# ariasanovsky/azdopt

Measured on AMD Instinct MI355X. Metric: node_expansions_per_s, higher is better.
Workload: dtype f32

## Files before the change

azdopt_amd/_lib.py:

```python
import ctypes as C
import os
import subprocess

_HERE = os.path.dirname(os.path.abspath(__file__))
LIB_PATH = os.environ.get("AZD_LIB", os.path.join(_HERE, "libazdopt_amd.so"))
_LIB = None

CTR = dict(EXPANSIONS=0, TERMINALS=1, TRANSPOSITIONS=2, VISITED_STEPS=3, SELECT_CALLS=4, SUM_DEG=5,
           SUM_ACTIONS=6, CASCADE_NODES=7, NEW_PREDS=8, ROOT_EXHAUSTED=9, MAX_FRONTIER=10, MAX_DEPTH=11,
           CURIOSITY_PAIRS=12, EVAL_LAYER_CLOCKS=13, TICKS_ADD_ACTIONS=14, FAILED=15, TICKS_TOTAL=16, TICKS_SELECT=17, TICKS_LOOKUP=18, TICKS_NEWNODE=19,
           TICKS_CASCADE=20, TICKS_MAX_CALL=21, TICKS_LAMBDA=22, TICKS_MATCHING=23, TICKS_WAIT=24, EVAL_BATCHES=25, EVAL_ROWS=26, EVAL_TILES=27, TICKS_TILES=28, TICKS_BATCH=29, TICKS_TILE_SETUP=30, TICKS_TILE_KLOOP=31)
CTR_COUNT = 32

ACT_NONE, ACT_RELU, ACT_SIGMOID = 0, 1, 2
ENGINE_NO_PERSISTENT_STEP = 1
ENGINE_ASYNC_STEP = 2
ENGINE_BARRIER_STEP = 4
ENGINE_POOL_STEP = 8
ENGINE_RAMSEY_U64 = 16
SPACE_C21 = 1
SPACE_RAMSEY = 2
SPACE_DENSE = 3
RAMSEY_MAX_N = 23
RAMSEY_WIDE_MAX_N = 32
# ... 57 lines not shown
    global _LIB
    if _LIB is not None:
        return _LIB
    if not os.path.exists(LIB_PATH):
        raise ImportError(f"{LIB_PATH} is missing: run __graft_entry__.build() (hipcc --offload-arch=gfx950); "
                          "azdopt_amd has no CPU fallback")
    L = C.CDLL(LIB_PATH)
    vp, i32p, u64p, f32p = C.c_void_p, C.POINTER(C.c_int32), C.POINTER(C.c_uint64), C.POINTER(C.c_float)

    def sig(name, res, *args):
        f = getattr(L, name, None)
        if f is None:
            if "AZD_LIB" in os.environ:
                return
            raise AttributeError("%s does not export %s" % (LIB_PATH, name))
        f.restype = res
        f.argtypes = list(args)

    sig("azd_status_string", C.c_char_p, C.c_int)
    sig("azd_last_error", C.c_char_p)
    sig("azd_version", C.c_int)
    sig("azd_device_count", C.c_int)
    sig("azd_c21_state_dim", C.c_int, C.c_int)
    sig("azd_c21_action_dim", C.c_int, C.c_int)
    sig("azd_c21_key_words", C.c_int, C.c_int)
    sig("azd_c21_generate_roots", C.c_int, C.c_uint64, C.c_uint64, C.c_uint64, C.c_int, C.c_int, C.c_int, C.c_int, vp, vp)
    sig("azd_evaluator_create_mlp", C.c_int, C.POINTER(vp), C.c_int, C.c_int, C.c_int, C.c_int, vp, C.c_int, C.c_int,
        C.POINTER(AdamConfig), C.c_uint64)
    sig("azd_evaluator_create_trivial", C.c_int, C.POINTER(vp), C.c_int, C.c_int, C.c_int)
    sig("azd_evaluator_create_hash_stream", C.c_int, C.POINTER(vp), C.c_int, C.c_int, C.c_int, C.c_uint64, C.c_uint64)
    sig("azd_evaluator_destroy", C.c_int, vp)
    sig("azd_evaluator_write_predictions", C.c_int, vp, C.c_int, vp, vp)
    sig("azd_evaluator_update_model", C.c_int, vp, C.c_int, vp, vp, vp, f32p)
    sig("azd_evaluator_write_predictions_dev", C.c_int, vp, C.c_int, vp, vp, vp)
    sig("azd_evaluator_update_model_dev", C.c_int, vp, C.c_int, vp, vp, vp, f32p, vp)
    sig("azd_evaluator_set_weight_storage", C.c_int, vp, C.c_int)
    sig("azd_evaluator_num_params", C.c_int64, vp)
    sig("azd_evaluator_get_params", C.c_int, vp, vp)
    sig("azd_evaluator_set_params", C.c_int, vp, vp)
    sig("azd_evaluator_calls", C.c_uint64, vp)
    sig("azd_engine_create", C.c_int, C.POINTER(vp), C.POINTER(EngineConfig), vp)
    sig("azd_engine_destroy", C.c_int, vp)
    sig("azd_engine_par_new", C.c_int, vp, vp, vp)
    sig("azd_engine_par_roll_out_episodes", C.c_int, vp, vp, C.c_int, C.c_uint32, C.c_int, i32p)
    sig("azd_engine_run_ahead", C.c_int, vp, vp, C.c_int, C.c_uint32, C.c_int, i32p)
    sig("azd_engine_par_update_model", C.c_int, vp, C.c_uint32, f32p)
    sig("azd_engine_par_update_model_sharded", C.c_int, vp, C.c_uint32, vp, f32p)
    sig("azd_engine_par_reset_trees", C.c_int, vp, vp, vp)
    sig("azd_engine_argmin_data", C.c_int, vp, C.POINTER(Argmin))
    sig("azd_engine_agent_counters", C.c_int, vp, vp)
    sig("azd_engine_agent_counters_per_agent", C.c_int, vp)
    sig("azd_engine_pool_agent_finish", C.c_int, vp, vp)
    sig("azd_engine_pool_groups", C.c_int, vp, vp, vp, vp)
    sig("azd_engine_ramsey_argmin_data", C.c_int, vp, C.POINTER(RamseyArgmin))
    sig("azd_engine_ramsey_wide_argmin_data", C.c_int, vp, C.POINTER(RamseyWideArgmin))
    sig("azd_engine_ramsey_argmin_any", C.c_int, vp, vp, C.c_int, vp, C.c_int, vp, f32p, i32p, C.POINTER(C.c_uint32))
    sig("azd_engine_ramsey_agent_counts", C.c_int, vp, C.c_int, vp, vp)
    sig("azd_ramsey_state_dim", C.c_int, C.c_int, C.c_int)
    sig("azd_ramsey_action_dim", C.c_int, C.c_int, C.c_int)
    sig("azd_ramsey_key_words", C.c_int, C.c_int, C.c_int)
    sig("azd_ramsey_generate_roots", C.c_int, C.c_uint64, C.c_uint64, C.c_uint64, C.c_int, C.c_int, C.c_int, C.c_int,
        C.c_int, vp, vp)
    sig("azd_dense_state_dim", C.c_int, C.c_int)
    sig("azd_dense_action_dim", C.c_int, C.c_int)
    sig("azd_dense_key_words", C.c_int, C.c_int)
    sig("azd_dense_generate_roots", C.c_int, C.c_uint64, C.c_uint64, C.c_uint64, C.c_int, C.c_int, C.c_int, C.c_int, C.c_double, vp, vp)
    sig("azd_engine_dense_argmin_data", C.c_int, vp, C.POINTER(DenseArgmin))
    sig("azd_c21_modify_roots", C.c_int, vp, C.c_uint64, C.c_uint64, C.c_int, C.c_int, vp, vp)
    sig("azd_c21_modify_roots_dev", C.c_int, vp, C.c_uint64, C.c_uint64, C.c_int, C.c_int, vp, vp)
    sig("azd_engine_par_reset_trees_c21", C.c_int, vp, C.c_uint64, C.c_uint64, C.c_int, C.c_int)
    sig("azd_engine_modify_roots_dev", C.c_int, vp, C.c_uint64, C.c_uint64, C.c_int, C.c_int, vp, vp)
    sig("azd_engine_par_reset_trees_policy", C.c_int, vp, C.c_uint64, C.c_uint64, C.c_int, C.c_int)
    sig("azd_engine_par_new_begin", C.c_int, vp, vp, vp)
    sig("azd_engine_par_new_end", C.c_int, vp, vp)
    sig("azd_engine_roll_out_begin", C.c_int, vp, vp, C.c_int, C.c_uint32)
    sig("azd_engine_roll_out_end", C.c_int, vp, vp, i32p)
    sig("azd_engine_reset_begin", C.c_int, vp, vp, vp)
    sig("azd_engine_reset_end", C.c_int, vp, vp)
    sig("azd_engine_observe", C.c_int, vp, C.c_uint32, vp, vp, vp)
    sig("azd_engine_observe_dev", C.c_int, vp, C.c_uint32, C.POINTER(vp), C.POINTER(vp), C.POINTER(vp))
    sig("azd_engine_read_state_vecs", C.c_int, vp, vp)
    sig("azd_engine_read_predictions", C.c_int, vp, vp)
    sig("azd_engine_debug_tile_forward", C.c_int, vp, vp, vp, C.c_int)
    sig("azd_engine_tree_sizes", C.c_int, vp, C.c_int, i32p, i32p, i32p)
    sig("azd_engine_export_tree", C.c_int, vp, C.c_int, *([vp] * 13))
    sig("azd_engine_agent_state", C.c_int, vp, C.c_int, vp, vp, vp, C.POINTER(C.c_uint32), C.POINTER(C.c_double), i32p)
    sig("azd_engine_counters", C.c_int, vp, vp)
    sig("azd_engine_set_timing", C.c_int, vp, C.c_int)
    sig("azd_engine_timing", C.c_int, vp, C.POINTER(C.c_double), C.POINTER(C.c_double), u64p)
    sig("azd_engine_stream", vp, vp)
    sig("azd_engine_step_form", C.c_int, vp, i32p, C.POINTER(C.c_char_p))
    sig("azd_engine_pool_split", C.c_int, vp, i32p, i32p)
    sig("azd_engine_pool_utilisation", C.c_int, vp, C.POINTER(C.c_double), C.POINTER(C.c_double))
    sig("azd_debug_probe_xcc", C.c_int, C.c_int, vp, C.c_int)
    sig("azd_debug_hash_stream_via_evaluators", C.c_int, vp, C.c_int)
    sig("azd_debug_mlp_gradients", C.c_int, vp, C.c_int, vp, vp, vp, vp, f32p)
    sig("azd_debug_probe_math", C.c_int, C.c_int, vp, vp, C.c_int)
    sig("azd_debug_gemm_bf16", C.c_int, C.c_int, C.c_int, C.c_int, C.c_int, vp, vp, vp, vp, C.c_int, C.c_int, C.c_int, C.c_int, f32p)
    sig("azd_debug_probe_cost", C.c_int, C.c_int, vp, C.c_int, C.c_int, C.c_int, C.c_int, vp, vp, f32p)
    _LIB = L
    return L


def check(status, where):
    if status != 0:
        raise AzdError(status, where)
# ... 5 lines not shown
```

azdopt_amd/csrc/engine.hip:

```cpp
#include <hip/hip_runtime.h>

#include <dlfcn.h>

#include <algorithm>
#include <cstdio>
#include <cstring>
#include <new>
#include <string>
#include <vector>

#include "../../include/azdopt_amd.h"
#include "c21_host.h"
#include "engine_types.h"
#include "evaluator.h"
#include "space_ops.h"

namespace azd {

thread_local std::string g_last_error;

int hip_fail(hipError_t e, const char *what) {
    g_last_error = std::string(what) + ": " + hipGetErrorString(e);
    if (e == hipErrorNoDevice || e == hipErrorInvalidDevice) return AZD_ERR_NO_DEVICE;
    if (e == hipErrorOutOfMemory) return AZD_ERR_OUT_OF_MEMORY;
// ... 112 lines not shown
    bool initialised = false;
    bool persist_enabled = true;
    bool barrier_step = false;
    azd::PersistArgs *d_pargs = nullptr;
    azd::PersistArgs *h_pargs = nullptr;
    azd::PersistArgs pargs_sent{};
    bool pargs_valid = false;
    bool log_clean = false;
    bool pool_clean = false;
    bool pool_failed = false;
    bool counters_by_wave = false;
    uint32_t *d_resume = nullptr;
    int16_t *d_grp_tile = nullptr;
    uint32_t *d_grp_lds = nullptr, *d_grp_desc = nullptr, *d_grp_cnt = nullptr, *d_grp_flag = nullptr;
    size_t grp_flag_words = 0;
    float *d_grp_x = nullptr;
    size_t grp_x_floats = 0, grp_slots_alloc = 0;
    std::vector<int16_t> grp_tile_host;
    std::vector<uint32_t> grp_lds_host;
    unsigned long long *d_log_key = nullptr;
    uint32_t *d_log_node = nullptr;
    int log_calls = 0;
    hipGraphExec_t call_graph = nullptr;
    azd::TolTable call_graph_tol{};
    uint64_t call_graph_layout = 0;
    bool graph_enabled = true;
    static constexpr int MAX_SUBS = 8;
    hipStream_t sub_stream[MAX_SUBS] = {};
    hipEvent_t sub_fork = nullptr, sub_join[MAX_SUBS] = {};
    hipGraphExec_t sub_graph[MAX_SUBS] = {};
    int sub_graph_n = 0;
    uint32_t *d_call_ctr = nullptr;
    static constexpr int EXT_STREAMS = 2;
    static constexpr int EXT_IN_FLIGHT = 4;
    hipStream_t ext_stream[EXT_STREAMS] = {};
    hipGraphExec_t ext_graph[EXT_STREAMS] = {};
    uint64_t ext_graph_layout = 0;
    int ext_graph_n = 0;
    bool ext_unsupported = false;
    uint32_t *d_ext_rows = nullptr, *d_ext_home = nullptr, *d_ext_n = nullptr;
    unsigned long long *d_ext_t0 = nullptr;
    int ext_depth = 2;
    hipEvent_t ext_done = nullptr, ext_fork = nullptr, ext_ring[EXT_STREAMS][EXT_IN_FLIGHT] = {};
    unsigned long long ext_iterations = 0;
    int kw_host = 0;
    int ramsey_slots = 0;
    int dense_slots = 0;
    uint64_t *d_stage_slots = nullptr;
    std::vector<uint64_t> dense_packed;
    std::vector<uint64_t> ramsey_perm_pad;
    bool pool_step = false;
    azd::PoolArgs pool{};
    size_t pool_slot_words = 0;
    int n_cus = 0;
    int pool_eval_wgs = 0, pool_search_wgs = 0;
    int pool_grp_g = 0, pool_grp_groups = 0, pool_grp_w = 0;
    int pool_search_waves = 0;
    double pool_util_eval = 0, pool_util_search = 0;
    struct {
        int n_eval = 0;
        int updates = 0;
    } pool_fb;
    struct Window {
        bool open = false;
        bool drained = false;
        bool lumped = false;
        int n = 0, consumed = 0;
        azd::TolTable tol{};
        uint32_t best_ord = 0;
        unsigned long long best_key = ~0ull;
        unsigned long long side_key = ~0ull;
        unsigned long long base_improved = 0;
        unsigned long long reported = 0;
        azd::FusedEval fe{};
        azd::PoolArgs pool{};
    } win;
    unsigned long long *h_win_log = nullptr;
    uint32_t *h_win_flag = nullptr;
    azd::ArgminRec *d_argmin_side = nullptr;
    azd::RamseyArgminRec *d_argmin_r_side = nullptr;
    bool ramsey_wide() const { return a.space == azd::SPACE_RAMSEY && a.KW > azd::MAX_KW; }
    bool ramsey_u64() const { return a.space == azd::SPACE_RAMSEY && a.KW == azd::RAMSEY_U64_KW; }
    size_t ramsey_nbr_words() const { return ramsey_u64() ? 512 : 128; }
    size_t argmin_r_bytes() const {
        return ramsey_u64() ? sizeof(azd::RamseyU64ArgminRec) : ramsey_wide() ? sizeof(azd::RamseyWideArgminRec) : sizeof(azd::RamseyArgminRec);
    }
    size_t argmin_r_recs() const { return (argmin_r_bytes() + sizeof(azd::RamseyArgminRec) - 1) / sizeof(azd::RamseyArgminRec); }
    float *d_pool = nullptr;
    size_t pool_rows = 0;
    int step_form = 0;
    std::string step_reason;

    template <typename T>
    int alloc(T **p, size_t count) {
        void *q = nullptr;
        hipError_t e = hipMalloc(&q, count * sizeof(T));
        if (e != hipSuccess) return azd::hip_fail(e, "hipMalloc");
        allocs.push_back(q);
        *p = (T *)q;
        return AZD_OK;
    }
    hipEvent_t get_event() {
        if (!ev_pool.empty()) {
            hipEvent_t e = ev_pool.back();
            ev_pool.pop_back();
            return e;
// ... 663 lines not shown
        TRY(e->alloc(&e->d_argmin_side, 1));
        if (ramsey) TRY(e->alloc(&e->d_argmin_r_side, e->argmin_r_recs()));
        hipError_t he3 = hipHostMalloc((void **)&e->h_win_log, (size_t)e->log_calls * sizeof(unsigned long long), hipHostMallocCoherent);
        if (he3 == hipSuccess) he3 = hipHostMalloc((void **)&e->h_win_flag, (size_t)e->log_calls * sizeof(uint32_t), hipHostMallocCoherent);
        if (he3 != hipSuccess) {
            st = azd::hip_fail(he3, "hipHostMalloc");
            azd_engine_destroy(e);
            return st;
        }
        e->pool.win_log = e->h_win_log;
        e->pool.win_flag = e->h_win_flag;
    }
    TRY(e->alloc(&e->d_stage_parents, B * (size_t)(dense ? 8 * a.n : ramsey ? a.E : a.n)));
    TRY(e->alloc(&e->d_stage_perm, B * (size_t)(dense ? 17 * a.KW : a.KW)));
    if (!dense) e->d_stage_slots = e->d_stage_perm;
    {
        hipError_t he = hipHostMalloc((void **)&e->h_status, sizeof(azd::StatusRec));
        if (he == hipSuccess) he = hipHostMalloc((void **)&e->h_argmin, sizeof(azd::ArgminRec));
        if (he != hipSuccess) {
            st = azd::hip_fail(he, "hipHostMalloc");
            azd_engine_destroy(e);
            return st;
        }
    }
    hipError_t he = hipMemsetAsync(a.counters, 0, B * azd::NUM_COUNTERS * 8, e->stream);
    if (he == hipSuccess) he = hipMemsetAsync(a.status, 0, sizeof(azd::StatusRec), e->stream);
    if (he == hipSuccess) he = hipMemsetAsync(a.argmin, 0, sizeof(azd::ArgminRec), e->stream);
    if (he == hipSuccess) he = hipMemsetAsync(a.flags, 0, B * 4, e->stream);
    if (he == hipSuccess) he = hipMemsetAsync(a.h_theta, 0, B * a.A * 4, e->stream);
    if (he == hipSuccess) he = hipMemsetAsync(a.state_vecs, 0, B * a.S * 4, e->stream);
    if (he == hipSuccess) he = hipMemsetAsync(a.weights, 0, B * a.A * 4, e->stream);
    if (he == hipSuccess) he = hipStreamSynchronize(e->stream);
    if (he != hipSuccess) {
        st = azd::hip_fail(he, "engine init memset");
        azd_engine_destroy(e);
        return st;
    }
#undef TRY
    *out = e;
    return AZD_OK;
}

int azd_engine_destroy(azd_engine *e) {
    if (!e) return AZD_OK;
    (void)hipSetDevice(e->cfg.device);
    if (e->stream) (void)hipStreamSynchronize(e->stream);
    for (void *p : e->allocs) (void)hipFree(p);
    if (e->h_status) (void)hipHostFree(e->h_status);
    if (e->h_argmin) (void)hipHostFree(e->h_argmin);
    if (e->h_pargs) (void)hipHostFree(e->h_pargs);
    if (e->h_win_log) (void)hipHostFree(e->h_win_log);
    if (e->h_win_flag) (void)hipHostFree(e->h_win_flag);
    if (e->d_pool) (void)hipFree(e->d_pool);
    for (void *p : {(void *)e->d_grp_tile, (void *)e->d_grp_lds, (void *)e->d_grp_desc, (void *)e->d_grp_cnt, (void *)e->d_grp_x, (void *)e->d_grp_flag})
        if (p) (void)hipFree(p);
    if (e->call_graph) (void)hipGraphExecDestroy(e->call_graph);
    for (int i = 0; i < azd_engine::MAX_SUBS; ++i) {
        if (e->sub_graph[i]) (void)hipGraphExecDestroy(e->sub_graph[i]);
        if (e->sub_join[i]) (void)hipEventDestroy(e->sub_join[i]);
        if (e->sub_stream[i]) (void)hipStreamDestroy(e->sub_stream[i]);
    }
    if (e->sub_fork) (void)hipEventDestroy(e->sub_fork);
    if (e->ext_done) (void)hipEventDestroy(e->ext_done);
    if (e->ext_fork) (void)hipEventDestroy(e->ext_fork);
    for (int x = 0; x < azd_engine::EXT_STREAMS; ++x) {
        if (e->ext_graph[x]) (void)hipGraphExecDestroy(e->ext_graph[x]);
        for (int i = 0; i < azd_engine::EXT_IN_FLIGHT; ++i)
            if (e->ext_ring[x][i]) (void)hipEventDestroy(e->ext_ring[x][i]);
        if (e->ext_stream[x]) (void)hipStreamDestroy(e->ext_stream[x]);
    }
    for (auto &it : e->ev_inflight) {
        (void)hipEventDestroy(it.second.first);
        (void)hipEventDestroy(it.second.second);
    }
    for (hipEvent_t ev : e->ev_pool) (void)hipEventDestroy(ev);
    if (e->stream) (void)hipStreamDestroy(e->stream);
    delete e;
    return AZD_OK;
}

int azd_engine_par_new_begin(azd_engine *e, const uint8_t *parents, const uint64_t *permitted) {
    if (!e || !parents || !permitted) return AZD_ERR_INVALID_ARGUMENT;
    AZD_ENTER(e);
    int st = upload_roots(e, parents, permitted);
    if (st) return st;
    const azd::Arenas &a = e->a;
    AZD_HIP(hipMemsetAsync(a.counters, 0, (size_t)a.B * azd::NUM_COUNTERS * 8, e->stream));
    e->counters_by_wave = false;
    AZD_HIP(hipMemsetAsync(a.status, 0, sizeof(azd::StatusRec), e->stream));
    e->seen_improved = 0;
    e->ops->init_roots(a, e->d_stage_parents, e->d_stage_perm, e->stream);
    AZD_HIP(hipMemsetAsync(a.h_theta, 0, (size_t)a.B * a.A * 4, e->stream));
    AZD_HIP(hipGetLastError());
    return AZD_OK;
}
static int new_finish(azd_engine *e) {
    e->ops->add_actions(e->a, 1, e->stream);
    e->ops->argmin(e->a, 1, e->stream);
    e->initialised = true;
    return sync_status(e);
}
int azd_engine_par_new_end(azd_engine *e, const float *h_theta) {
    if (!e || !h_theta) return AZD_ERR_INVALID_ARGUMENT;
    AZD_ENTER(e);
    AZD_HIP(hipMemcpyAsync(e->a.h_theta, h_theta, (size_t)e->a.B * e->a.A * 4, hipMemcpyHostToDevice, e->stream));
    return new_finish(e);
}
// ... 47 lines not shown
        tiles[l] = (fe.dims[l + 1] + 15) / 16;
        max_tiles = std::max(max_tiles, tiles[l]);
        if (l < L - 1) xs = std::max<uint32_t>(xs, (uint32_t)tiles[l] * 256u);
        if (l < L - 1 && fe.dims[l + 1] % 16 != 0) return false;
    }
    for (int W : {1, 2, 4})
    for (int g = force_g > 0 ? force_g : 8; g <= avail_wgs && g <= 128; g += 8) {
        {
            if (force_g <= 0 && W < 4 && 2 * g > avail_wgs) break;
            if ((max_tiles + g - 1) / g > W) {
                if (force_g > 0) break;
                continue;
            }
            struct Item { int l, t; size_t bytes; };
            std::vector<Item> items;
            for (int l = 0; l < L; ++l)
                for (int t = 0; t < tiles[l]; ++t) items.push_back({l, t, (size_t)steps[l] * 1024});
            std::stable_sort(items.begin(), items.end(), [](const Item &x, const Item &y) { return x.bytes > y.bytes; });
            std::vector<size_t> load((size_t)g, 0);
            std::vector<int> cnt((size_t)L * g, 0);
            std::vector<int16_t> tile((size_t)L * g * W, (int16_t)-1);
            std::vector<uint32_t> lds((size_t)L * g * W, 0u);
            bool ok = true;
            for (const Item &it : items) {
                int best = -1;
                for (int m = 0; m < g; ++m)
                    if (cnt[(size_t)it.l * g + m] < W && (best < 0 || load[(size_t)m] < load[(size_t)best])) best = m;
                if (best < 0 || load[(size_t)best] + it.bytes > lds_budget) {
                    ok = false;
                    break;
                }
                const int w = cnt[(size_t)it.l * g + best]++;
                tile[((size_t)it.l * g + best) * W + w] = (int16_t)it.t;
                lds[((size_t)it.l * g + best) * W + w] = (uint32_t)load[(size_t)best];
                load[(size_t)best] += it.bytes;
            }
            if (!ok) {
                if (force_g > 0) break;
                continue;
            }
            out->g = g;
            out->W = W;
            out->lds_bytes = *std::max_element(load.begin(), load.end());
            out->xstride = xs ? xs : 256u;
            out->tile = tile;
            out->lds = lds;
            return true;
        }
        if (force_g > 0) break;
    }
    return false;
}

static int pool_clear(azd_engine *e, const azd::PoolArgs &pool) {
    AZD_HIP(hipMemsetAsync(pool.ctl, 0, sizeof(azd::PoolCtl), e->stream));
    AZD_HIP(hipMemsetAsync(pool.ready_slots, 0, e->pool_slot_words * sizeof(uint32_t), e->stream));
    AZD_HIP(hipMemsetAsync(pool.join, 0, (size_t)e->a.B * sizeof(uint32_t), e->stream));
    e->pool_clean = true;
    return AZD_OK;
}

static int pool_finish_launch(azd_engine *e, const azd::FusedEval &fe, const azd::PoolArgs &pool, int k, bool *took_over,
                              uint32_t *as_out, size_t *ab_out) {
    *took_over = false;
    int st = fetch_status(e);
    if (st) return st;
    if (e->h_status->pool_ticks > 0 && !e->h_status->pool_abort) {
        const double T = (double)e->h_status->pool_ticks;
        e->pool_util_eval = e->pool_eval_wgs > 0 ? (double)e->h_status->pool_eval_busy / (T * e->pool_eval_wgs) : 0.0;
        e->pool_util_search = e->pool_search_waves > 0 ? (double)e->h_status->pool_search_busy / (T * e->pool_search_waves) : 0.0;
    }
    if (!e->h_status->pool_abort) return AZD_OK;
    e->pool_clean = false;
    e->log_clean = false;
    e->pool_failed = true;
    e->pool_step = false;
    uint32_t as = 0;
    size_t ab = 0;
    const char *why_t = "";
    if (!e->ops->async_plan(e->a, fe, &as, &ab, &why_t)) {
        e->time_collect();
        azd::g_last_error = std::string("pool step: a queue wait ran into its bound, and the asynchronous step cannot take over: ") + why_t;
        return AZD_ERR_UNREACHABLE;
    }
    azd::launch_pool_resume_scan(e->a, pool, k, e->d_resume, e->stream);
    st = pool_clear(e, pool);
    if (st) return st;
    azd::StepLaunch sl;
    sl.n_calls = k;
    sl.log_key = e->d_log_key;
    sl.resume = e->d_resume;
    sl.ctl = nullptr;
    sl.hashed = fe.kind == 4;
    sl.window = 0;
    e->time_begin(0);
    e->ops->launch_async(e->a, e->d_pargs, sl, fe.params, fe.wpk, as, ab, e->stream);
    e->time_end();
    e->log_clean = true;
    e->step_form = AZD_STEP_ASYNC;
    e->step_reason = "pool step aborted (a queue wait ran into its bound: no evaluator or searcher workgroup made progress); "
                     "the asynchronous step took the launch over and serves this engine from here on";
    *took_over = true;
    *as_out = as;
    *ab_out = ab;
    return AZD_OK;
}

static int dense_pool_run(azd_engine *e, const azd::TolTable &t, int n_calls, bool *ran, int *left_out) {
    *ran = false;
    *left_out = 0;
// ... 372 lines not shown
            if (const char *env = getenv("AZD_POOL_EVAL_GROUP")) {
                force_g = atoi(env);
                want = force_g > 0;
            }
            GroupPlan gpl;
            const int avail = capacity - n_search;
            if (want && plan_groups(fe, (size_t)160 * 1024 - 2048, avail, force_g, &gpl)) {
                const int n_groups = std::max(1, avail / gpl.g);
                const int NS = 16 / gpl.W;
                const size_t slots = (size_t)n_groups * NS;
                if (!e->d_grp_tile) {
                    AZD_HIP(hipMalloc(&e->d_grp_tile, (size_t)8 * 128 * 4 * sizeof(int16_t)));
                    AZD_HIP(hipMalloc(&e->d_grp_lds, (size_t)8 * 128 * 4 * sizeof(uint32_t)));
                }
                if (slots > e->grp_slots_alloc || slots * 2 * gpl.xstride > e->grp_x_floats || slots * gpl.g * 16 > e->grp_flag_words) {
                    AZD_HIP(hipStreamSynchronize(e->stream));
                    (void)hipFree(e->d_grp_desc);
                    (void)hipFree(e->d_grp_cnt);
                    (void)hipFree(e->d_grp_x);
                    (void)hipFree(e->d_grp_flag);
                    e->d_grp_flag = nullptr;
                    e->d_grp_desc = e->d_grp_cnt = nullptr;
                    e->d_grp_x = nullptr;
                    AZD_HIP(hipMalloc(&e->d_grp_desc, slots * 64 * 4));
                    AZD_HIP(hipMalloc(&e->d_grp_cnt, slots * 8 * 32 * 4));
                    AZD_HIP(hipMalloc(&e->d_grp_x, slots * 2 * gpl.xstride * 4));
                    AZD_HIP(hipMalloc(&e->d_grp_flag, slots * gpl.g * 16 * 4));
                    e->grp_flag_words = slots * gpl.g * 16;
                    e->grp_slots_alloc = slots;
                    e->grp_x_floats = slots * 2 * gpl.xstride;
                }
                if (gpl.tile != e->grp_tile_host || gpl.lds != e->grp_lds_host) {
                    AZD_HIP(hipStreamSynchronize(e->stream));
                    AZD_HIP(hipMemcpy(e->d_grp_tile, gpl.tile.data(), gpl.tile.size() * sizeof(int16_t), hipMemcpyHostToDevice));
                    AZD_HIP(hipMemcpy(e->d_grp_lds, gpl.lds.data(), gpl.lds.size() * sizeof(uint32_t), hipMemcpyHostToDevice));
                    e->grp_tile_host = gpl.tile;
                    e->grp_lds_host = gpl.lds;
                }
                pool.grp_g = gpl.g;
                pool.grp_w = gpl.W;
                pool.grp_groups = n_groups;
                pool.grp_tile = e->d_grp_tile;
                pool.grp_lds = e->d_grp_lds;
                pool.grp_desc = e->d_grp_desc;
                pool.grp_cnt = e->d_grp_cnt;
                pool.grp_x = e->d_grp_x;
                pool.grp_flag = e->d_grp_flag;
                pool.grp_xstride = gpl.xstride;
                n_eval = n_groups * gpl.g;
                pool.n_eval = n_eval;
                if (gpl.lds_bytes > dyn_bytes) dyn_bytes = gpl.lds_bytes;
            }
        }
        pool_blocks = n_eval + n_search;
        e->pool_grp_g = pool.grp_g;
        e->pool_grp_groups = pool.grp_groups;
        e->pool_grp_w = pool.grp_w;
        e->pool_eval_wgs = n_eval;
        e->pool_search_wgs = n_search;
        e->pool_search_waves = (n_search - pool.n_express) * 16 + pool.n_express * (int)pool.express_waves;
    }
    if (e->pool_step && fusable && !use_pool) {
        use_async = !e->barrier_step && e->ops->async_plan(e->a, fe, &dyn_stride, &dyn_bytes, &why_a);
        use_barrier = !use_async && e->ops->persist_plan(e->a, fe, &dyn_stride, &dyn_bytes, &why_b);
        if (!use_async) e->step_reason += why_a;
        if (!use_async && !use_barrier && *why_b) e->step_reason += std::string("; ") + why_b;
    }
    e->step_form = use_pool ? AZD_STEP_POOL : use_async ? AZD_STEP_ASYNC : use_barrier ? AZD_STEP_BARRIER : AZD_STEP_PER_CALL;
    if (e->a.space == azd::SPACE_DENSE)
        e->step_reason = dense_reason.empty() ? "AZD_DENSE_NO_POOL: the dense-graph space's pool step was switched off" : dense_reason;
    if (ahead) {
        const bool ok = use_pool && fe.kind >= 3 && n_calls >= 1 && n_calls <= e->log_calls && !e->timing;
        if (!ok) return AZD_OK;
        *accepted = 1;
    }
    if (use_pool || use_async || use_barrier) {
        auto send_args = [&](const azd::PoolArgs &pl) -> int {
            azd::PersistArgs &pa = e->pargs_sent;
            azd::PersistArgs now;
            memset(&now, 0, sizeof(now));
            now.a = e->a;
            now.tol = t;
            now.ev = fe;
            now.ev.call_base = (fe.kind == 2 || fe.kind == 4) ? e->ev->calls : 0;
            now.pool = pl;
            if (e->pargs_valid && memcmp(&pa, &now, sizeof(now)) == 0) return AZD_OK;
            AZD_HIP(hipStreamSynchronize(e->stream));
            memcpy(e->h_pargs, &now, sizeof(now));
            AZD_HIP(hipMemcpyAsync(e->d_pargs, e->h_pargs, sizeof(azd::PersistArgs), hipMemcpyHostToDevice, e->stream));
            memcpy(&pa, &now, sizeof(now));
            e->pargs_valid = true;
            return AZD_OK;
        };
        const bool fb_on = use_pool && fe.kind == 3 && pool_feedback_on() && n_calls >= 100 && !getenv("AZD_POOL_EVAL_WGS");
        int left = n_calls;
        while (left > 0) {
            const int k = left < e->log_calls ? left : e->log_calls;
            status_fresh = false;
            st = send_args(pool);
            if (st) return st;
            if (use_pool && !e->pool_clean) {
                st = pool_clear(e, pool);
                if (st) return st;
            }
            if (use_pool && pool.grp_g > 0) {
                const size_t slots = (size_t)pool.grp_groups * (16 / pool.grp_w);
// ... 658 lines not shown
    return AZD_OK;
}
int azd_engine_ramsey_agent_counts(azd_engine *e, int agent, int32_t *counts, int32_t *totals) {
    if (!e || agent < 0 || agent >= e->a.B) return AZD_ERR_INVALID_ARGUMENT;
    if (e->a.space != azd::SPACE_RAMSEY) return AZD_ERR_UNSUPPORTED;
    AZD_ENTER(e);
    AZD_HIP(hipStreamSynchronize(e->stream));
    const azd::Arenas &a = e->a;
    if (counts) AZD_HIP(hipMemcpy(counts, a.cur_counts + (size_t)agent * a.C * a.E, (size_t)a.C * a.E * 4, hipMemcpyDeviceToHost));
    if (totals) AZD_HIP(hipMemcpy(totals, a.cur_tot + (size_t)agent * 4, 16, hipMemcpyDeviceToHost));
    return AZD_OK;
}

int azd_engine_argmin_data(azd_engine *e, azd_argmin *out) {
    if (!e || !out || !e->initialised) return AZD_ERR_INVALID_ARGUMENT;
    if (e->a.space != azd::SPACE_C21) return AZD_ERR_UNSUPPORTED;
    AZD_HIP(hipSetDevice(e->cfg.device));
    bool side = false;
    {
        const int st_w = window_argmin_side(e, &side);
        if (st_w) return st_w;
    }
    static_assert(sizeof(azd_argmin) == sizeof(azd::ArgminRec), "ABI struct mismatch");
    AZD_HIP(hipMemcpyAsync(e->h_argmin, side ? e->d_argmin_side : e->a.argmin, sizeof(azd::ArgminRec), hipMemcpyDeviceToHost, e->stream));
    AZD_HIP(hipStreamSynchronize(e->stream));
    memcpy(out, e->h_argmin, sizeof(azd_argmin));
    return AZD_OK;
}

int azd_engine_read_state_vecs(azd_engine *e, float *out) {
    if (!e || !out) return AZD_ERR_INVALID_ARGUMENT;
    AZD_ENTER(e);
    AZD_HIP(hipStreamSynchronize(e->stream));
    AZD_HIP(hipMemcpy(out, e->a.state_vecs, (size_t)e->a.B * e->a.S * 4, hipMemcpyDeviceToHost));
    return AZD_OK;
}
int azd_engine_debug_tile_forward(azd_engine *e, const float *states, float *predictions, int rows) {
    if (!e || !states || !predictions || rows < 1) return AZD_ERR_INVALID_ARGUMENT;
    AZD_ENTER(e);
    azd::FusedEval fe;
    azd::PoolArgs pool = e->pool;
    uint32_t dyn_stride = 0;
    size_t dyn_bytes = 0;
    const char *why = "";
    if (e->a.space == azd::SPACE_DENSE || !e->ev->fused_desc(&fe) || fe.kind != 3 || !e->ops->pool_plan(e->a, fe, &pool, &dyn_stride, &dyn_bytes, &why)) {
        azd::g_last_error = "debug_tile_forward: needs the c21 or the Ramsey space with an MLP evaluator the pool step can serve";
        return AZD_ERR_INVALID_ARGUMENT;
    }
    float *d_in = nullptr, *d_out = nullptr;
    hipError_t he = hipMalloc(&d_in, (size_t)rows * e->a.S * 4);
    const char *what = "hipMalloc";
    if (he == hipSuccess) he = hipMalloc(&d_out, (size_t)rows * e->a.A * 4);
    if (he == hipSuccess) what = "hipMemcpyAsync", he = hipMemcpyAsync(d_in, states, (size_t)rows * e->a.S * 4, hipMemcpyHostToDevice, e->stream);
    if (he == hipSuccess) what = "k_tile_forward", he = azd::launch_tile_forward(fe, pool, rows, d_in, d_out, e->stream);
    if (he == hipSuccess) what = "hipMemcpyAsync", he = hipMemcpyAsync(predictions, d_out, (size_t)rows * e->a.A * 4, hipMemcpyDeviceToHost, e->stream);
    if (he == hipSuccess) what = "hipStreamSynchronize", he = hipStreamSynchronize(e->stream);
    else (void)hipStreamSynchronize(e->stream);
    (void)hipFree(d_in);
    (void)hipFree(d_out);
    return he == hipSuccess ? AZD_OK : azd::hip_fail(he, what);
}
int azd_engine_read_predictions(azd_engine *e, float *out) {
    if (!e || !out) return AZD_ERR_INVALID_ARGUMENT;
    AZD_ENTER(e);
    AZD_HIP(hipStreamSynchronize(e->stream));
    AZD_HIP(hipMemcpy(out, e->a.h_theta, (size_t)e->a.B * e->a.A * 4, hipMemcpyDeviceToHost));
    return AZD_OK;
}

int azd_engine_tree_sizes(azd_engine *e, int agent, int *n_nodes, int *n_arcs, int *n_preds) {
    if (!e || agent < 0 || agent >= e->a.B) return AZD_ERR_INVALID_ARGUMENT;
    AZD_ENTER(e);
    AZD_HIP(hipStreamSynchronize(e->stream));
    uint32_t v[3];
    AZD_HIP(hipMemcpy(&v[0], e->a.n_nodes + agent, 4, hipMemcpyDeviceToHost));
    AZD_HIP(hipMemcpy(&v[1], e->a.n_arcs + agent, 4, hipMemcpyDeviceToHost));
    AZD_HIP(hipMemcpy(&v[2], e->a.n_preds + agent, 4, hipMemcpyDeviceToHost));
    if (n_nodes) *n_nodes = (int)v[0];
    if (n_arcs) *n_arcs = (int)v[1];
    if (n_preds) *n_preds = (int)v[2];
    return AZD_OK;
}

int azd_engine_export_tree(azd_engine *e, int agent, float *c, float *c_star, uint32_t *n_t, uint32_t *exhausted,
                           uint32_t *act_begin, uint32_t *act_end, uint64_t *keys, uint32_t *arc_src,
                           uint32_t *arc_dst, uint32_t *arc_pp, uint32_t *pred_a_id, float *pred_g,
                           int32_t *pred_arc) {
    int nn, na, np;
    int st = azd_engine_tree_sizes(e, agent, &nn, &na, &np);
    if (st) return st;
    const azd::Arenas &a = e->a;
    std::vector<azd::NodeRec> nodes((size_t)nn);
    std::vector<azd::ArcRec> arcs((size_t)na);
    std::vector<azd::PredRec> preds((size_t)np);
    AZD_HIP(hipMemcpy(nodes.data(), a.nodes + (size_t)agent * a.node_cap, nodes.size() * sizeof(azd::NodeRec), hipMemcpyDeviceToHost));
    if (na) AZD_HIP(hipMemcpy(arcs.data(), a.arcs + (size_t)agent * a.arc_cap, arcs.size() * sizeof(azd::ArcRec), hipMemcpyDeviceToHost));
    if (np) AZD_HIP(hipMemcpy(preds.data(), a.preds + (size_t)agent * a.pred_cap, preds.size() * sizeof(azd::PredRec), hipMemcpyDeviceToHost));
    std::vector<float> g_exp((size_t)np);
    if (np) AZD_HIP(hipMemcpy(g_exp.data(), a.pred_g + (size_t)agent * a.pred_cap, g_exp.size() * 4, hipMemcpyDeviceToHost));
    if (keys && a.space == azd::SPACE_DENSE) {
        const int KW = a.KW, MAXS = e->dense_slots;
        std::vector<uint64_t> rk((size_t)nn * KW);
        std::vector<uint16_t> tab((size_t)MAXS);
        AZD_HIP(hipMemcpy(rk.data(), a.keys + (size_t)agent * a.node_cap * KW, rk.size() * 8, hipMemcpyDeviceToHost));
        AZD_HIP(hipMemcpy(tab.data(), a.root_aid + (size_t)agent * MAXS, tab.size() * 2, hipMemcpyDeviceToHost));
        memset(keys, 0, (size_t)nn * e->kw_host * 8);
        for (int i = 0; i < nn; ++i)
// ... 95 lines not shown
    if (!e || !out) return AZD_ERR_INVALID_ARGUMENT;
    AZD_ENTER(e);
    AZD_HIP(hipStreamSynchronize(e->stream));
    const azd::Arenas &a = e->a;
    std::vector<unsigned long long> h((size_t)a.B * azd::NUM_COUNTERS);
    std::vector<uint32_t> fl((size_t)a.B);
    AZD_HIP(hipMemcpy(h.data(), a.counters, h.size() * 8, hipMemcpyDeviceToHost));
    AZD_HIP(hipMemcpy(fl.data(), a.flags, fl.size() * 4, hipMemcpyDeviceToHost));
    for (int k = 0; k < AZD_CTR_COUNT; ++k) out[k] = 0;
    for (int i = 0; i < a.B; ++i) {
        for (int k = 0; k < azd::NUM_COUNTERS; ++k) {
            unsigned long long v = h[(size_t)i * azd::NUM_COUNTERS + k];
            if (k >= AZD_CTR_COUNT) continue;
            if (k == AZD_CTR_MAX_FRONTIER || k == AZD_CTR_MAX_DEPTH || k == AZD_CTR_TICKS_MAX_CALL) out[k] = std::max<uint64_t>(out[k], v);
            else out[k] += v;
        }
    }
    uint64_t failed = 0;
    for (uint32_t f : fl) failed += f != 0;
    out[AZD_CTR_FAILED_AGENTS] = failed;
    return AZD_OK;
}

int azd_engine_agent_counters(azd_engine *e, uint64_t *out) {
    if (!e || !out) return AZD_ERR_INVALID_ARGUMENT;
    AZD_ENTER(e);
    AZD_HIP(hipStreamSynchronize(e->stream));
    AZD_HIP(hipMemcpy(out, e->a.counters, (size_t)e->a.B * azd::NUM_COUNTERS * 8, hipMemcpyDeviceToHost));
    return AZD_OK;
}
int azd_engine_agent_counters_per_agent(azd_engine *e) { return e ? (e->counters_by_wave ? 0 : 1) : AZD_ERR_INVALID_ARGUMENT; }

int azd_engine_set_timing(azd_engine *e, int enabled) {
    if (!e) return AZD_ERR_INVALID_ARGUMENT;
    e->timing = enabled != 0;
    e->rollout_ms = e->evaluator_ms = 0;
    e->rollout_launches = 0;
    return AZD_OK;
}
int azd_engine_timing(azd_engine *e, double *tree_ms, double *evaluator_ms, uint64_t *tree_launches) {
    if (!e) return AZD_ERR_INVALID_ARGUMENT;
    if (tree_ms) *tree_ms = e->rollout_ms;
    if (evaluator_ms) *evaluator_ms = e->evaluator_ms;
    if (tree_launches) *tree_launches = e->rollout_launches;
    return AZD_OK;
}
void *azd_engine_stream(azd_engine *e) { return e ? (void *)e->stream : nullptr; }
int azd_engine_pool_utilisation(azd_engine *e, double *eval_busy, double *search_busy) {
    if (!e) return AZD_ERR_INVALID_ARGUMENT;
    if (eval_busy) *eval_busy = e->pool_util_eval;
    if (search_busy) *search_busy = e->pool_util_search;
    return AZD_OK;
}
int azd_engine_pool_groups(azd_engine *e, int *members, int *groups, int *waves_per_slot) {
    if (!e) return AZD_ERR_INVALID_ARGUMENT;
    if (members) *members = e->pool_grp_g;
    if (groups) *groups = e->pool_grp_groups;
    if (waves_per_slot) *waves_per_slot = e->pool_grp_w;
    return AZD_OK;
}
int azd_engine_pool_agent_finish(azd_engine *e, uint64_t *ticks_out) {
    if (!e || !ticks_out) return AZD_ERR_INVALID_ARGUMENT;
    AZD_ENTER(e);
    if (!e->pool.stamp) {
        azd::g_last_error = "pool_agent_finish: this engine has run no pool step";
        return AZD_ERR_INVALID_ARGUMENT;
    }
    AZD_HIP(hipStreamSynchronize(e->stream));
    AZD_HIP(hipMemcpy(ticks_out, e->pool.stamp, (size_t)e->a.B * 8, hipMemcpyDeviceToHost));
    return AZD_OK;
}
int azd_engine_pool_split(azd_engine *e, int *eval_wgs, int *search_wgs) {
    if (!e) return AZD_ERR_INVALID_ARGUMENT;
    if (eval_wgs) *eval_wgs = e->pool_eval_wgs;
    if (search_wgs) *search_wgs = e->pool_search_wgs;
    return AZD_OK;
}
int azd_debug_probe_xcc(int device, uint32_t *out, int n_blocks) {
    if (!out || n_blocks <= 0) return AZD_ERR_INVALID_ARGUMENT;
    int st = azd::device_ok(device);
    if (st) return st;
    AZD_HIP(hipSetDevice(device));
    uint32_t *d = nullptr;
    AZD_HIP(hipMalloc(&d, (size_t)n_blocks * 4));
    azd::launch_probe_xcc(d, n_blocks, nullptr);
    hipError_t he = hipDeviceSynchronize();
    if (he == hipSuccess) he = hipMemcpy(out, d, (size_t)n_blocks * 4, hipMemcpyDeviceToHost);
    (void)hipFree(d);
    if (he != hipSuccess) return azd::hip_fail(he, "probe_xcc");
    return AZD_OK;
}
int azd_engine_step_form(azd_engine *e, int *form, const char **reason) {
    if (!e) return AZD_ERR_INVALID_ARGUMENT;
    if (form) *form = e->step_form;
    if (reason) *reason = e->step_reason.c_str();
    return AZD_OK;
}

int azd_debug_probe_math(int device, const float *in, float *out, int n) {
    if (!in || !out || n <= 0) return AZD_ERR_INVALID_ARGUMENT;
    int st = azd::device_ok(device);
    if (st) return st;
    AZD_HIP(hipSetDevice(device));
    float *d_in = nullptr, *d_out = nullptr;
    AZD_HIP(hipMalloc(&d_in, (size_t)n * 8));
    AZD_HIP(hipMalloc(&d_out, (size_t)n * 16));
// ... 149 lines not shown
```

azdopt_amd/csrc/engine_types.h:

```cpp
#pragma once
#include <stddef.h>
#include <stdint.h>

namespace azd {

constexpr uint32_t NONE = 0xFFFFFFFFu;
constexpr int PARENTS_STRIDE = 32;
constexpr int MAX_N = 24;
constexpr int MAX_KW = 6;
constexpr int PATH_SET = 0, PATH_SEQUENCE = 1;
constexpr int SPACE_C21 = 1, SPACE_RAMSEY = 2, SPACE_DENSE = 3;
constexpr int PRED_CHUNKS = 2;
constexpr int MAX_NODE_ACTIONS = 64 * PRED_CHUNKS;
constexpr int RAMSEY_U64_KW = 36;
constexpr int RAMSEY_U64_CH = 8;
constexpr int FRONTIER_CAP = 256;
constexpr int PATH_STACK = 32;
constexpr int MAX_TOL = 32;
constexpr int NUM_COUNTERS = 32;

struct __attribute__((aligned(16))) NodeRec {
    float c_star;
    uint32_t nt_ex;
    float c;
// ... 162 lines not shown
struct FusedEval {
    int kind;
    uint64_t seed, first_agent, call_base;
    const float *params;
    int n_layers;
    int dims[8];
    int final_act;
    int max_hidden;
    int hid[2];
    long long w_off[7], b_off[7];
    int bf16;
    const uint16_t *w16;
    const void *wpk;
    long long p_off[7];
};

struct TolTable {
    uint32_t tol[MAX_TOL];
    int n_tol;
    uint32_t tol_default;
};

constexpr int POOL_XCDS = 8;
struct PoolQ {
    uint32_t head, pad0[31];
    uint32_t tail, pad1[31];
};
struct PoolCtl {
    uint32_t claim_next, pad0[31];
    uint32_t done_agents, pad1[31];
    uint32_t abort, pad2[31];
    PoolQ ready[2][POOL_XCDS];
    PoolQ evalq[2][POOL_XCDS];
    struct {
        uint32_t v, pad[31];
    } sum_calls[POOL_XCDS], claimed[POOL_XCDS],
      done_x[POOL_XCDS],
      max_lag[POOL_XCDS];
    unsigned long long eval_busy;
    unsigned long long search_busy;
    unsigned long long t_first;
    unsigned long long t_last;
};
struct PendRec {
    uint32_t pos;
    float c;
    uint32_t n_preds;
    uint32_t call;
};
struct PoolArgs {
    PoolCtl *ctl;
    uint32_t *ready_slots;
    uint32_t *eval_slots;
    int ready_lanes;
    int n_express;
    uint32_t express_waves;
    uint32_t express_shift;
    int early_post;
    uint32_t qcap;
    uint32_t *join;
    PendRec *pend;
    unsigned long long *stamp;
    int n_eval;
    uint32_t eval_stride;
    uint32_t eval_out_off;
    uint32_t eval_rows;
    uint32_t *post_call;
    int grp_g, grp_w, grp_groups;
    const int16_t *grp_tile;
    const uint32_t *grp_lds;
    uint32_t *grp_desc;
    uint32_t *grp_cnt;
    uint32_t *grp_flag;
    float *grp_x;
    uint32_t grp_xstride;
    uint32_t debug_abort_call;
    uint32_t *win_count;
    unsigned long long *win_log;
    uint32_t *win_flag;
};

struct StepLaunch {
    int n_calls;
    unsigned long long *log_key;
    const uint32_t *resume;
    PoolCtl *ctl;
    int hashed;
    int groups = 0;
    int window;
};

struct PersistArgs {
    Arenas a;
    TolTable tol;
    FusedEval ev;
    PoolArgs pool;
};

}
```

azdopt_amd/csrc/pool_kernels.hip:

```cpp
#define AZD_TU_ASYNC 1
#define AZD_TU_POOL 1
#include <hip/hip_runtime.h>

#include "bf16.h"
#include "c21_host.h"
#include "space_ops.h"

namespace azd {

#include "tree_core.inc"
#include "space_c21.inc"
#include "persistent_step.inc"
#include "async_step.inc"
#include "pool_step.inc"
#include "launchers.inc"

static bool e_pool_plan(const Arenas &a, const FusedEval &ev, PoolArgs *pool, uint32_t *dyn_stride, size_t *dyn_bytes, const char **why) {
    return pool_plan_common(a, ev, pool, dyn_stride, dyn_bytes, why, C21Space<1>::pool_dyn_bytes(a), sizeof(WaveLds));
}
static void e_launch_pool(const Arenas &a, const PersistArgs *d_args, const StepLaunch &sl, const float *params,
                          const void *wpk, int n_blocks, uint32_t dyn_stride, size_t dyn_bytes, void *stream) {
    DISPATCH_KW(a, l_pool, a, d_args, sl, params, wpk, n_blocks, dyn_stride, dyn_bytes, (hipStream_t)stream);
}
static int e_pool_max_resident(const Arenas &a, size_t dyn_bytes, int n_cus) {
    int nb = 0;
    DISPATCH_KW(a, q_pool_resident, &nb, dyn_bytes);
    return nb * n_cus;
}
const PoolOps &c21_pool_ops() {
    static const PoolOps ops = {e_pool_plan, e_launch_pool, e_pool_max_resident};
    return ops;
}

__global__ __launch_bounds__(PERSIST_WAVES * 64) void k_tile_forward(const FusedEval ev, const float *__restrict__ params, const void *__restrict__ wpk,
                                                                     const uint32_t stride, const uint32_t out_off, const int n_rows,
                                                                     const float *__restrict__ states, float *__restrict__ out) {
    __shared__ uint32_t agents[PERSIST_WAVES];
    const int tid = threadIdx.x, wave = tid >> 6, first = blockIdx.x * PERSIST_WAVES;
    const int n = n_rows - first < PERSIST_WAVES ? n_rows - first : PERSIST_WAVES;
    const int S = ev.dims[0], S16 = (S + 15) & ~15, L = ev.n_layers, A = ev.dims[L];
    if (tid < PERSIST_WAVES) agents[tid] = (uint32_t)(first + tid);
    PoolRows rows;
    rows.stride = stride;
    rows.out_off = out_off;
    rows.agents = agents;
    rows.n = n;
    EvalPtrs gp;
    gp.params = params;
    gp.wpk = wpk;
    gp.state_vecs = states;
    gp.h_theta = out;
    for (int idx = tid; idx < n * S16; idx += PERSIST_WAVES * 64) {
        const int r = idx / S16, c = idx - r * S16;
        const float v = c < S ? states[(size_t)(first + r) * S + c] : 0.f;
        if (ev.bf16) reinterpret_cast<uint16_t *>(rows.row(r))[c] = (uint16_t)bf16_bits(v);
        else rows.row(r)[c] = v;
    }
    __syncthreads();
    for (int l = 0; l < L; ++l) {
        const int nt = (ev.dims[l + 1] + 15) >> 4;
        for (int tile = wave; tile < nt; tile += PERSIST_WAVES) {
            unsigned long long ph[3];
            mlp_tile_task<PoolRows, true>(ev, rows, gp, l, tile, ph);
        }
        __syncthreads();
    }
    for (int idx = tid; idx < n * A; idx += PERSIST_WAVES * 64) {
        const int r = idx / A, c = idx - r * A;
        out[(size_t)(first + r) * A + c] = rows.out(r)[c];
    }
}
hipError_t launch_tile_forward(const FusedEval &ev, const PoolArgs &pool, int n_rows, const float *states, float *out, void *stream) {
    const size_t dyn_bytes = (size_t)pool.eval_stride * sizeof(float) * PERSIST_WAVES;
    hipError_t he = hipFuncSetAttribute((const void *)k_tile_forward, hipFuncAttributeMaxDynamicSharedMemorySize, (int)dyn_bytes);
    if (he != hipSuccess) return he;
    k_tile_forward<<<dim3((n_rows + PERSIST_WAVES - 1) / PERSIST_WAVES), dim3(PERSIST_WAVES * 64), dyn_bytes, (hipStream_t)stream>>>(
        ev, ev.params, ev.wpk, pool.eval_stride, pool.eval_out_off, n_rows, states, out);
    return hipGetLastError();
}
__global__ void k_pool_resume_scan(Arenas a, const PendRec *__restrict__ pend, const uint32_t *__restrict__ claim_next, const int n_calls,
                                   uint32_t *__restrict__ resume) {
    const int t = blockIdx.x * blockDim.x + threadIdx.x;
    if (t >= a.B) return;
    const uint32_t claimed = *claim_next;
    uint32_t r = 0u;
    if ((uint32_t)t < claimed) {
        const NodeRec nd = a.nodes[(size_t)t * a.node_cap + a.state_pos[t]];
        const bool pending = a.flags[t] == 0u && nd.act_end == 0u;
        r = pending ? (pend[t].call | 0x80000000u) : (uint32_t)n_calls;
    }
    resume[t] = r;
}
void launch_pool_resume_scan(const Arenas &a, const PoolArgs &pool, int n_calls, uint32_t *resume, void *stream) {
    k_pool_resume_scan<<<dim3((a.B + 255) / 256), dim3(256), 0, (hipStream_t)stream>>>(a, pool.pend, &pool.ctl->claim_next, n_calls, resume);
}
__global__ void k_probe_xcc(uint32_t *out) {
    if (threadIdx.x == 0) out[blockIdx.x] = pool_xcc_id();
}
void launch_probe_xcc(uint32_t *d_out, int n_blocks, void *stream) {
    k_probe_xcc<<<dim3(n_blocks), dim3(64), 0, (hipStream_t)stream>>>(d_out);
}

}
```

azdopt_amd/csrc/pool_step.inc:

```

constexpr unsigned long long POOL_WAIT_TICKS = 400000000ull;
struct PoolWait {
    unsigned long long t0;
    uint32_t polls;
    __device__ __forceinline__ PoolWait() : t0(0), polls(0) {}
    __device__ __forceinline__ bool expired() {
        if ((++polls & 255u) != 0u) return false;
        const unsigned long long now = (unsigned long long)wall_clock64();
        if (t0 == 0) t0 = now;
        return now - t0 > POOL_WAIT_TICKS;
    }
};

__device__ __forceinline__ uint32_t pool_xcc_id() {
    uint32_t v;
    asm volatile("s_getreg_b32 %0, hwreg(HW_REG_XCC_ID)" : "=s"(v));
    return v & 7u;
}

#ifndef AZD_POOL_FILL_WAIT
#define AZD_POOL_FILL_WAIT 2
#endif
#ifndef AZD_POOL_FILL_SLEEP
#define AZD_POOL_FILL_SLEEP 32
// ... 135 lines not shown
__device__ __forceinline__ int opaque_lane() {
    int v;
    asm volatile("v_mbcnt_lo_u32_b32 %0, -1, 0\n\tv_mbcnt_hi_u32_b32 %0, -1, %0" : "=v"(v));
    return v;
}
__device__ __forceinline__ void pool_tile1(const FusedEval &ev, const PoolRows &rows, const EvalPtrs &gp, const int l, const int tile) {
    const int L = ev.n_layers;
    const int K = ev.dims[l], N = ev.dims[l + 1];
    const int S4 = (ev.dims[0] + 15) & ~15, H = ev.hid[0];
    const int nrows = rows.count();
    const int n0 = tile * 16;
    const int steps = (K + 15) >> 4;
    const size_t tile0 = (size_t)ev.p_off[l] + (size_t)tile * steps * 256;
    azd_tile_acc acc = {0.f, 0.f, 0.f, 0.f};
    {
        const int lane = opaque_lane();
        const int r = lane & 15;
        float *const rbase = rows.row(r < nrows ? r : 0);
        const int in_off = (l == 0 ? 0 : S4 + ((l - 1) & 1) * H) + 4 * (lane >> 4);
        if (ev.bf16)
            tile_k_loop_bf16(acc, reinterpret_cast<const uint16_t *>(gp.wpk) + tile0, (uint32_t)lane * 8u,
                             (uint32_t)(uintptr_t)(reinterpret_cast<const uint16_t *>(rbase) + in_off), steps);
        else
            tile_k_loop_f32(acc, reinterpret_cast<const float *>(gp.wpk) + tile0, (uint32_t)lane * 16u, (uint32_t)(uintptr_t)(rbase + in_off), steps);
    }
    const int lane = opaque_lane();
    const int col = n0 + (lane & 15);
    if (col < N) {
        const float bj = gp.params[ev.b_off[l] + col];
        const int act = (l == L - 1) ? ev.final_act : 1;
#pragma unroll
        for (int i = 0; i < 4; ++i) {
            const int row = 4 * (lane >> 4) + i;
            if (row < nrows) {
                const float v = act_apply(acc[i] + bj, act);
                if (l == L - 1) rows.out(row)[col] = v;
                else if (ev.bf16) reinterpret_cast<uint16_t *>(rows.row(row))[S4 + (l & 1) * H + col] = (uint16_t)bf16_bits(v);
                else rows.row(row)[S4 + (l & 1) * H + col] = v;
            }
        }
    }
}

__device__ __forceinline__ void pool_hash_rows(const FusedEval &ev, const PoolArgs &pl, const PoolBatch &bt, const PoolRows &rows, const int n,
                                            const int A) {
    for (int idx = threadIdx.x; idx < n * A; idx += PERSIST_WAVES * 64) {
        const int r = idx / A, i = idx - r * A;
        const uint64_t agent = ev.first_agent + (uint64_t)bt.agent[r], cidx = ev.call_base + (uint64_t)ld_sc1(pl.post_call + bt.agent[r]);
        const uint64_t h = splitmix(splitmix(splitmix(splitmix(ev.seed ^ 0x70726564ull) ^ agent) ^ cidx) ^ (uint64_t)i);
        rows.out(r)[i] = (float)(h >> 40) * (1.0f / 16777216.0f);
    }
}

template <bool HASHED>
__device__ __forceinline__ void pool_eval(const PersistArgs *pa, const EvalPtrs &gp, PoolBatch &bt, const uint32_t xcc) {
    const Arenas &a = pa->a;
    const FusedEval &ev = pa->ev;
    const PoolArgs &pl = pa->pool;
    PoolCtl *ctl = pl.ctl;
    const int tid = threadIdx.x, wave = tid >> 6;
    const uint32_t B = (uint32_t)a.B, qmask = pl.qcap - 1u;
    constexpr bool hashed = HASHED;
    const int S = ev.dims[0], S16 = (S + 15) & ~15, L = hashed ? 0 : ev.n_layers, A = hashed ? a.A : ev.dims[L];
    PoolRows rows;
    rows.stride = pl.eval_stride;
    rows.out_off = pl.eval_out_off;
    rows.agents = bt.agent;
    unsigned long long n_batches = 0, n_rows = 0, n_tiles = 0, busy = 0, t_stage = 0, t_layers = 0, c_layers = 0;
    for (;;) {
        if (tid == 0) {
            uint32_t n = 0, first0 = 0, first1 = 0, cnt0 = 0, cnt1 = 0, q = 0, leave = 0;
            PoolWait wt;
            int fill_waits = AZD_POOL_FILL_WAIT;
            for (;;) {
                for (uint32_t k = 0; k < (uint32_t)POOL_XCDS && n == 0u; ++k) {
                    const uint32_t x = (xcc + k) & (uint32_t)(POOL_XCDS - 1);
                    const uint32_t h0 = AZD_POOL_PRIORITY ? ld_sc1(&ctl->evalq[0][x].head) : 0u, t0 = AZD_POOL_PRIORITY ? ld_sc1(&ctl->evalq[0][x].tail) : 0u;
                    const uint32_t h1 = ld_sc1(&ctl->evalq[1][x].head), t1 = ld_sc1(&ctl->evalq[1][x].tail);
                    const int a0 = (int)(t0 - h0) > 0 ? (int)(t0 - h0) : 0, a1 = (int)(t1 - h1) > 0 ? (int)(t1 - h1) : 0;
                    if (a0 + a1 == 0) continue;
                    const int cap = ((int)pl.eval_rows > PERSIST_WAVES && a0 + a1 >= (int)pl.eval_rows) ? (int)pl.eval_rows : PERSIST_WAVES;
                    if (a0 == 0 && a1 < PERSIST_WAVES && fill_waits > 0) {
                        --fill_waits;
                        __builtin_amdgcn_s_sleep(AZD_POOL_FILL_SLEEP);
                        k = (uint32_t)POOL_XCDS;
                        continue;
                    }
                    uint32_t c0 = 0, c1 = 0;
                    if (a0 > 0) {
                        const uint32_t take = a0 < cap ? (uint32_t)a0 : (uint32_t)cap;
                        if (atomicCAS(&ctl->evalq[0][x].head, h0, h0 + take) == h0) c0 = take;
                    }
                    if (a1 > 0 && c0 < (uint32_t)cap) {
                        const uint32_t room = (uint32_t)cap - c0;
                        const uint32_t take = (uint32_t)a1 < room ? (uint32_t)a1 : room;
                        if (atomicCAS(&ctl->evalq[1][x].head, h1, h1 + take) == h1) c1 = take;
                    }
                    if (c0 + c1) {
                        n = c0 + c1;
                        first0 = h0;
                        first1 = h1;
                        cnt0 = c0;
                        cnt1 = c1;
                        q = x;
                    } else k = (uint32_t)POOL_XCDS;
                }
                if (n) break;
                if (ld_sc1(&ctl->done_agents) >= B || ld_sc1(&ctl->abort) != 0u) {
                    leave = 1;
                    break;
                }
                __builtin_amdgcn_s_sleep(AZD_POOL_EVAL_IDLE_SLEEP);
                if (wt.expired()) {
                    atomicExch(&ctl->abort, 1u);
                    leave = 1;
                    break;
                }
            }
            bt.n = n;
            bt.first[0] = first0;
            bt.first[1] = first1;
            bt.cnt[0] = cnt0;
            bt.cnt[1] = cnt1;
            bt.q = q;
            bt.leave = leave;
        }
        __syncthreads();
        if (bt.leave) break;
        const int n = (int)bt.n;
        const unsigned long long tb0 = (unsigned long long)wall_clock64();
        if (tid < n) {
            const uint32_t lane_q = (uint32_t)tid < bt.cnt[0] ? 0u : 1u;
            const uint32_t ticket = lane_q == 0u ? bt.first[0] + (uint32_t)tid : bt.first[1] + (uint32_t)tid - bt.cnt[0];
            uint32_t *slot = pl.eval_slots + ((size_t)lane_q * POOL_XCDS + bt.q) * pl.qcap + (ticket & qmask);
            uint32_t v = 0;
            PoolWait wt;
            while ((v = ld_sc1(slot)) == 0u) {
                __builtin_amdgcn_s_sleep(1);
                if (wt.expired() || ld_sc1(&ctl->abort) != 0u) {
                    atomicExch(&ctl->abort, 1u);
                    bt.leave = 1u;
                    break;
                }
            }
            st_sc1(slot, 0u);
            bt.agent[tid] = v ? (v & 0xFFFFFFu) - 1u : 0u;
            bt.home[tid] = v >> 24;
#ifdef AZD_PHASE_PROFILE
            if (v) {
                unsigned long long *st = pl.stamp + bt.agent[tid];
                atomicAdd(&a.counters[(size_t)bt.agent[tid] * NUM_COUNTERS + 24], (unsigned long long)wall_clock64() - __hip_atomic_load(st, __ATOMIC_RELAXED, __HIP_MEMORY_SCOPE_AGENT));
            }
#endif
        }
        __syncthreads();
        if (bt.leave) break;
        rows.n = n;
        if (hashed) pool_hash_rows(ev, pl, bt, rows, n, A);
        else {
            const int q4 = S16 >> 2;
            for (int idx = tid; idx < n * q4; idx += PERSIST_WAVES * 64) {
                const int r = idx / q4, c4 = idx - r * q4;
                azd_f32x4 v = {0.f, 0.f, 0.f, 0.f};
                if (4 * c4 < S) v = ld_sc1_x4(gp.state_vecs + (size_t)bt.agent[r] * S + 4 * c4);
                if (ev.bf16) {
                    uint16_t *d = reinterpret_cast<uint16_t *>(rows.row(r)) + 4 * c4;
                    d[0] = (uint16_t)bf16_bits(v[0]);
                    d[1] = (uint16_t)bf16_bits(v[1]);
                    d[2] = (uint16_t)bf16_bits(v[2]);
                    d[3] = (uint16_t)bf16_bits(v[3]);
                } else *reinterpret_cast<azd_f32x4 *>(rows.row(r) + 4 * c4) = v;
            }
        }
        __syncthreads();
        const unsigned long long tb1 = (unsigned long long)wall_clock64();
        const unsigned long long cb1 = (unsigned long long)__builtin_amdgcn_s_memtime();
        for (int l = 0; l < L; ++l) {
            const int nt = (ev.dims[l + 1] + 15) >> 4;
            for (int tile = wave; tile < nt; tile += PERSIST_WAVES) {
                if (n > PERSIST_WAVES) {
                    if (ev.bf16) pool_tile2<true>(ev, rows, gp, l, tile);
                    else pool_tile2<false>(ev, rows, gp, l, tile);
                } else {
#if AZD_POOL_ASM_TILE
                    pool_tile1(ev, rows, gp, l, tile);
#else
                    unsigned long long ph[3];
                    mlp_tile_task<PoolRows, true>(ev, rows, gp, l, tile, ph);
#endif
                }
            }
            __syncthreads();
        }
        for (int l = 0; l < L; ++l) n_tiles += (unsigned long long)((ev.dims[l + 1] + 15) >> 4);
        const unsigned long long tb2 = (unsigned long long)wall_clock64();
        t_stage += tb1 - tb0;
        t_layers += tb2 - tb1;
        c_layers += (unsigned long long)__builtin_amdgcn_s_memtime() - cb1;
        {
            const int a4 = A >> 2;
            for (int idx = tid; idx < n * a4; idx += PERSIST_WAVES * 64) {
                const int r = idx / a4, c4 = idx - r * a4;
                st_sc1_x4(gp.h_theta + (size_t)bt.agent[r] * A + 4 * c4, *reinterpret_cast<const azd_f32x4 *>(rows.out(r) + 4 * c4));
            }
        }
        VM_DRAIN();
        __syncthreads();
        if (tid < n && ((bt.home[tid] & 0x40u) == 0u || (atomicAdd(&pl.join[bt.agent[tid]], 1u) & 1u))) {
#ifdef AZD_PHASE_PROFILE
            __hip_atomic_store(pl.stamp + bt.agent[tid], (unsigned long long)wall_clock64(), __ATOMIC_RELAXED, __HIP_MEMORY_SCOPE_AGENT);
#endif
            const uint32_t x = bt.home[tid] & (uint32_t)(POOL_XCDS - 1);
            const uint32_t rl = (pl.ready_lanes && (bt.home[tid] & 0x80u)) ? 0u : 1u;
            const uint32_t i = atomicAdd(&ctl->ready[rl][x].tail, 1u);
            st_sc1(pl.ready_slots + ((size_t)rl * POOL_XCDS + x) * pl.qcap + (i & qmask), bt.agent[tid] + 1u);
        }
        n_batches += 1;
        n_rows += (unsigned long long)n;
        if (tid == 0 && blockIdx.x == 0 && pl.debug_abort_call != 0u && n_batches == (unsigned long long)pl.debug_abort_call) atomicExch(&ctl->abort, 1u);
        busy += (unsigned long long)wall_clock64() - tb0;
    }
    if (tid == 0) {
        atomicAdd(&ctl->eval_busy, busy);
        atomicMax(&ctl->t_last, (unsigned long long)wall_clock64());
        unsigned long long *ctr = a.counters + (size_t)(blockIdx.x % (uint32_t)a.B) * NUM_COUNTERS;
        atomicAdd(&ctr[25], n_batches);
        atomicAdd(&ctr[26], n_rows);
// ... 250 lines not shown
                if (v >= gen && v != 0xFFFFFFFFu) break;
                __builtin_amdgcn_s_sleep(2);
                if (wt.expired() || ((wt.polls & 63u) == 0u && ld_sc1(&ctl->abort) != 0u)) {
                    atomicExch(&ctl->abort, 1u);
                    leave = true;
                    break;
                }
            }
            if (leave) {
                tell_all(7, 0xFFFFFFFFu);
                break;
            }
            n_batches += 1;
            n_rows += (unsigned long long)n;
            for (int l = 0; l < L; ++l) n_tiles += (unsigned long long)((ev.dims[l + 1] + 15) >> 4);
            busy += (unsigned long long)wall_clock64() - tb0;
            if (lane == 0 && si == 0 && pl.debug_abort_call != 0u && n_batches == (unsigned long long)pl.debug_abort_call) atomicExch(&ctl->abort, 1u);
        }
    }
    if (leader && lane == 0) {
        atomicAdd(&ctl->eval_busy, busy);
        atomicMax(&ctl->t_last, (unsigned long long)wall_clock64());
        unsigned long long *ctr = a.counters + (size_t)((blockIdx.x * PERSIST_WAVES + (uint32_t)wave) % (uint32_t)a.B) * NUM_COUNTERS;
        atomicAdd(&ctr[25], n_batches);
        atomicAdd(&ctr[26], n_rows);
        atomicAdd(&ctr[27], n_tiles);
        atomicAdd(&ctr[29], busy);
    }
}

struct PoolIdle {
    uint32_t leave;
    uint32_t claims_done;
    uint32_t mean_calls;
};

__device__ __forceinline__ void pool_window_count(const PoolArgs &pl, const unsigned long long *log_key, const uint32_t call, const uint32_t B) {
    if (atomicAdd(pl.win_count + call, 1u) + 1u != B) return;
    const unsigned long long key = __hip_atomic_load(log_key + call, __ATOMIC_RELAXED, __HIP_MEMORY_SCOPE_AGENT);
    __hip_atomic_store(pl.win_log + call, key, __ATOMIC_RELAXED, __HIP_MEMORY_SCOPE_SYSTEM);
    __hip_atomic_store(pl.win_flag + call, 1u, __ATOMIC_RELEASE, __HIP_MEMORY_SCOPE_SYSTEM);
}

template <class SP, int MODE>
__device__ __forceinline__ void pool_search(const PersistArgs *pa, const int n_calls, unsigned long long *__restrict__ log_key, typename SP::Lds &s,
                            const uint32_t dyn, const uint32_t xcc, PoolIdle &idle, const bool express) {
    const Arenas &a = pa->a;
    const TolTable &tol = pa->tol;
    const FusedEval &ev = pa->ev;
    const PoolArgs &pl = pa->pool;
    PoolCtl *ctl = pl.ctl;
    constexpr bool HASHED = (MODE & 1) != 0, WINDOW = (MODE & 2) != 0;
    const uint32_t B = (uint32_t)a.B, qmask = pl.qcap - 1u;
    uint32_t *rslots[2] = {pl.ready_slots + (size_t)xcc * pl.qcap, pl.ready_slots + ((size_t)POOL_XCDS + xcc) * pl.qcap};
    uint32_t *eslots[2] = {pl.eval_slots + (size_t)xcc * pl.qcap, pl.eval_slots + ((size_t)POOL_XCDS + xcc) * pl.qcap};
    for (;;) {
#ifdef AZD_WAVE_PHASES
        const unsigned long long wp_take0 = PH_NOW();
#endif
        uint32_t t = NONE, pending = 0, waited = 0;
        if (LANE == 0) {
            if (!express && LDS_LOAD(&idle.claims_done) == 0u) {
                const uint32_t c = atomicAdd(&ctl->claim_next, 1u);
                if (c < B) {
                    t = c;
                    atomicAdd(&ctl->claimed[xcc].v, 1u);
#ifdef AZD_PHASE_PROFILE
                    a.counters[(size_t)c * NUM_COUNTERS + 31] = (unsigned long long)wall_clock64();
#endif
                } else LDS_STORE(&idle.claims_done, 1u);
            }
            if (t == NONE && LDS_LOAD(&idle.leave) == 0u) {
                uint32_t rl = 1u;
                if (pl.ready_lanes == 1 && (int)(ld_sc1(&ctl->ready[0][xcc].head) - ld_sc1(&ctl->ready[0][xcc].tail)) < AZD_POOL_STANDBY) rl = 0u;
                if (express) rl = 0u;
                else if (pl.ready_lanes == 2 && (int)(ld_sc1(&ctl->ready[0][xcc].tail) - ld_sc1(&ctl->ready[0][xcc].head)) > 0) rl = 0u;
                const uint32_t h = atomicAdd(&ctl->ready[rl][xcc].head, 1u);
                uint32_t *slot = rslots[rl] + (h & qmask);
                PoolWait wt;
                uint32_t v = 0, polls = 0, seen_progress = 0xFFFFFFFFu;
                while ((v = ld_sc1(slot)) == 0u) {
                    if ((++polls & 15u) == 0u) {
                        if (LDS_LOAD(&idle.leave) != 0u) break;
                        if (ld_sc1(&ctl->done_agents) >= B || ld_sc1(&ctl->abort) != 0u) {
                            LDS_STORE(&idle.leave, 1u);
                            break;
                        }
                    }
                    __builtin_amdgcn_s_sleep(AZD_POOL_POLL_SLEEP);
#ifdef AZD_POOL_POLL_SLEEP2
                    __builtin_amdgcn_s_sleep(AZD_POOL_POLL_SLEEP2);
#endif
                    if (wt.expired()) {
                        uint32_t progress = 0u;
                        for (int x = 0; x < POOL_XCDS; ++x) progress += ld_sc1(&ctl->sum_calls[x].v);
                        if (progress != seen_progress) {
                            seen_progress = progress;
                            wt = PoolWait();
                        } else {
                            atomicExch(&ctl->abort, 1u);
                            LDS_STORE(&idle.leave, 1u);
                            break;
                        }
                    }
                }
                if (v) {
                    st_sc1(slot, 0u);
                    if ((h & 7u) == 0u || express) {
// ... 10 lines not shown
            }
        }
        t = uni(t);
        pending = uni(pending);
        waited = uni(waited);
        if (t == NONE) break;
        __builtin_amdgcn_fence(__ATOMIC_ACQUIRE, "agent");
#ifdef AZD_PHASE_PROFILE
        if (LANE < 24) s.ctr[LANE] = 0;
#endif
        if (LANE == 0) s.ctr[31] = (unsigned long long)wall_clock64();
#ifdef AZD_WAVE_PHASES
        CTR_ADD(24, PH_NOW() - wp_take0);
        const unsigned long long wp_add0 = PH_NOW();
#endif
        WAVE_SYNC();
        uint32_t call = 0u;
        RolloutOut first;
        first.first_nact = 0u;
        if (pending) {
#ifdef AZD_PHASE_PROFILE
            CTR_ADD(28, (unsigned long long)wall_clock64() - __hip_atomic_load(pl.stamp + t, __ATOMIC_RELAXED, __HIP_MEMORY_SCOPE_AGENT));
#endif
            const PendRec pr = pl.pend[t];
            RolloutOut ro;
            ro.flags = 0;
            ro.cand_c = 0.f;
            ro.cand_node = NONE;
            ro.pos = pr.pos;
            ro.c = pr.c;
            ro.n_preds = pr.n_preds;
            call = pr.call;
            add_actions_agent<SP, true>(a, s, (int)t, 0, &ro, &first);
#ifdef AZD_WAVE_PHASES
            CTR_ADD(14, PH_NOW() - wp_add0);
#endif
        }
        bool posted = false;
        for (;; ++call) {
            if (call >= (uint32_t)n_calls) {
                if (LANE == 0) {
                    atomicAdd(&ctl->done_agents, 1u);
                    if (pl.ready_lanes == 2) atomicAdd(&ctl->done_x[xcc].v, 1u);
#ifdef AZD_PHASE_PROFILE
                    a.counters[(size_t)t * NUM_COUNTERS + 30] = (unsigned long long)wall_clock64();
#else
                    pl.stamp[t] = (unsigned long long)wall_clock64() - __hip_atomic_load(&ctl->t_first, __ATOMIC_RELAXED, __HIP_MEMORY_SCOPE_AGENT);
#endif
                }
                break;
            }
            RolloutOut ro;
            ro.post_tail = nullptr;
            ro.posted = 0u;
            ro.known_live = first.first_nact != 0u ? 1u : 0u;
            ro.first_nact = first.first_nact;
            ro.first_pp = first.first_pp;
            ro.first_aid = first.first_aid;
            ro.first_g = first.first_g;
            first.first_nact = 0u;
            uint32_t behind = 0u, lane_q = 1u;
            if (HASHED || ev.kind == 3) {
#if AZD_POOL_PRIORITY
                {
                    const uint32_t cl = ld_sc1(&ctl->claimed[xcc].v);
                    const uint32_t mean = ld_sc1(&ctl->sum_calls[xcc].v) / (cl ? cl : 1u);
                    const uint32_t slack = (mean >> 5) > 2u ? (mean >> 5) : 2u;
                    if (call + 1u + slack < mean) lane_q = 0u;
                }
#endif
                if (pl.ready_lanes == 2) {
                    const uint32_t ref = LDS_LOAD(&idle.mean_calls);
                    if (call + (uint32_t)AZD_POOL_EXPRESS_SLACK + (ref >> pl.express_shift) < ref) behind = 0x80u;
                } else if (pl.ready_lanes) {
                    const uint32_t cl = ld_sc1(&ctl->claimed[xcc].v);
                    const uint32_t mean = ld_sc1(&ctl->sum_calls[xcc].v) / (cl ? cl : 1u);
                    behind = call + 1u + (uint32_t)AZD_POOL_READY_SLACK < mean ? 0x80u : 0u;
                }
                bool early = pl.early_post == 1;
                if (pl.early_post == 2) {
                    const uint32_t mean = LDS_LOAD(&idle.mean_calls);
                    early = waited || behind != 0u || call + (uint32_t)AZD_POOL_BEHIND_SLACK + (mean >> AZD_POOL_BEHIND_SHIFT) < mean;
                }
                ro.post_tail = early ? &ctl->evalq[lane_q][xcc].tail : nullptr;
                ro.post_slots = eslots[lane_q];
                ro.post_mask = qmask;
                ro.post_word = (t + 1u) | ((xcc | behind | 0x40u) << 24);
                ro.post_stamp = pl.stamp + t;
                if (HASHED && LANE == 0) st_sc1(pl.post_call + t, call);
            }
#ifdef AZD_WAVE_PHASES
            const unsigned long long wp_roll0 = PH_NOW();
#endif
            const bool expanded = rollout_agent<SP, true, true>(a, tol, s, dyn, (int)t, &ro);
#ifdef AZD_WAVE_PHASES
            CTR_ADD(28, PH_NOW() - wp_roll0);
#endif
            if (LANE == 0 && ro.flags == 0) {
                const uint32_t node = ro.cand_node;
                if (node != NONE) {
                    const unsigned long long key = ((unsigned long long)ordf(ro.cand_c) << 32) |
                                                   ((unsigned long long)(t & 0xFFFFu) << 16) | (unsigned long long)(node & 0xFFFFu);
                    atomicMin(&log_key[call], key);
                    a.cand_node[t] = NONE;
                }
            }
            if (LANE == 0) atomicAdd(&ctl->sum_calls[xcc].v, 1u);
            if (!expanded) {
                if (WINDOW) {
                    VM_DRAIN();
                    if (LANE == 0) pool_window_count(pl, log_key, call, B);
                }
                continue;
            }
            if (HASHED || ev.kind == 3) {
                if (LANE == 0) {
                    PendRec pr;
                    pr.pos = ro.pos;
                    pr.c = ro.c;
                    pr.n_preds = ro.n_preds;
                    pr.call = call + 1u;
                    pl.pend[t] = pr;
                }
                WAVE_SYNC();
                POOL_FLUSH_PER_AGENT(a, s, (int)t);
                VM_DRAIN();
                if (LANE == 0) {
                    if (!ro.posted) {
#ifdef AZD_PHASE_PROFILE
                        __hip_atomic_store(pl.stamp + t, (unsigned long long)wall_clock64(), __ATOMIC_RELAXED, __HIP_MEMORY_SCOPE_AGENT);
#endif
                        const uint32_t i = atomicAdd(&ctl->evalq[lane_q][xcc].tail, 1u);
                        st_sc1(eslots[lane_q] + (i & qmask), (t + 1u) | ((xcc | behind) << 24));
                    }
                    else if (atomicAdd(&pl.join[t], 1u) & 1u) {
#ifdef AZD_PHASE_PROFILE
                        __hip_atomic_store(pl.stamp + t, (unsigned long long)wall_clock64(), __ATOMIC_RELAXED, __HIP_MEMORY_SCOPE_AGENT);
#endif
                        const uint32_t rl = (pl.ready_lanes && behind) ? 0u : 1u;
                        const uint32_t i = atomicAdd(&ctl->ready[rl][xcc].tail, 1u);
                        st_sc1(rslots[rl] + (i & qmask), t + 1u);
                    }
                    if (WINDOW) pool_window_count(pl, log_key, call, B);
                }
                posted = true;
                break;
            }
            if (ev.kind == 2) {
                float *h = a.h_theta + (size_t)t * a.A;
                const uint64_t agent = ev.first_agent + (uint64_t)t, cidx = ev.call_base + (uint64_t)call;
                for (int i = LANE; i < a.A; i += 64) {
                    uint64_t r = splitmix(splitmix(splitmix(splitmix(ev.seed ^ 0x70726564ull) ^ agent) ^ cidx) ^ (uint64_t)i);
                    h[i] = (float)(r >> 40) * (1.0f / 16777216.0f);
                }
                WAVE_SYNC();
            }
            add_actions_agent<SP, false>(a, s, (int)t, 0, &ro, &first);
        }
        if (!posted) {
            WAVE_SYNC();
            POOL_FLUSH_PER_AGENT(a, s, (int)t);
        }
        if (LANE == 0) s.ctr[30] += (unsigned long long)wall_clock64() - s.ctr[31];
    }
    if (LANE == 0) {
        atomicAdd(&ctl->search_busy, s.ctr[30]);
        atomicMax(&ctl->t_last, (unsigned long long)wall_clock64());
    }
#ifndef AZD_PHASE_PROFILE
    WAVE_SYNC();
#ifdef AZD_WAVE_PHASES
    if ((LANE == 24 || LANE == 28) && s.ctr[LANE]) atomicAdd(&a.counters[(size_t)((blockIdx.x * PERSIST_WAVES + (threadIdx.x >> 6)) % B) * NUM_COUNTERS + LANE], s.ctr[LANE]);
#endif
    if (LANE < 24) {
        const unsigned long long v = s.ctr[LANE];
        unsigned long long *ctr = a.counters + (size_t)((blockIdx.x * PERSIST_WAVES + (threadIdx.x >> 6)) % B) * NUM_COUNTERS;
        if (LANE == 10 || LANE == 11 || LANE == 21) atomicMax(&ctr[LANE], v);
        else if (v) atomicAdd(&ctr[LANE], v);
    }
#endif
#ifdef AZD_PHASE_PROFILE
    if (LANE == 0 && s.ctr[28]) atomicAdd(&a.counters[(size_t)((blockIdx.x * PERSIST_WAVES + (threadIdx.x >> 6)) % B) * NUM_COUNTERS + 28], s.ctr[28]);
#endif
}

template <class SP, int MODE>
__global__ __launch_bounds__(PERSIST_WAVES * 64) void k_pool(const PersistArgs *__restrict__ pa, int n_calls,
                                                             unsigned long long *__restrict__ log_key, uint32_t dyn_stride,
                                                             const float *__restrict__ params, const float *state_vecs,
                                                             float *h_theta, const void *__restrict__ wpk) {
    constexpr uint32_t SW_BYTES = (uint32_t)((PERSIST_WAVES * sizeof(typename SP::Lds) + 15) & ~(size_t)15);
    typename SP::Lds *const sw = reinterpret_cast<typename SP::Lds *>(lds_base(0u));
    __shared__ PoolBatch bt;
    __shared__ PoolIdle idle;
    const uint32_t xcc = pool_xcc_id();
    if (threadIdx.x == 0) atomicCAS(&pa->pool.ctl->t_first, 0ull, (unsigned long long)wall_clock64());
    if ((int)blockIdx.x < pa->pool.n_eval) {
        EvalPtrs gp;
        gp.params = params;
        gp.wpk = wpk;
        gp.state_vecs = state_vecs;
        gp.h_theta = h_theta;
        if constexpr ((MODE & 4) != 0) {
            if (pa->pool.grp_g > 0 && (int)blockIdx.x < pa->pool.grp_groups * pa->pool.grp_g) {
                pool_eval_group(pa, gp, xcc);
                return;
            }
        }
        pool_eval<(MODE & 1) != 0>(pa, gp, bt, xcc);
        return;
    }
    const int wave = threadIdx.x >> 6;
    typename SP::Lds &s = sw[wave];
    if (threadIdx.x == 0) {
        idle.leave = 0u;
        idle.claims_done = 0u;
        idle.mean_calls = 0u;
    }
    SP::prepare(pa->a, s);
    if (LANE < NUM_COUNTERS) s.ctr[LANE] = 0;
    __syncthreads();
#ifdef AZD_POOL_ACTIVE_WAVES
    if (wave >= AZD_POOL_ACTIVE_WAVES) return;
#endif
    const bool express = pa->pool.ready_lanes == 2 && (int)blockIdx.x >= (int)gridDim.x - pa->pool.n_express;
    if (express && (uint32_t)wave >= pa->pool.express_waves) return;
    pool_search<SP, MODE>(pa, n_calls, log_key, s, SW_BYTES + (uint32_t)wave * dyn_stride, xcc, idle, express);
}

template <class SP, int MODE>
__global__ __launch_bounds__(PERSIST_WAVES * 64) void k_pool_search(const PersistArgs *__restrict__ pa, int n_calls,
                                                                    unsigned long long *__restrict__ log_key, uint32_t dyn_stride) {
    constexpr uint32_t SW_BYTES = (uint32_t)((PERSIST_WAVES * sizeof(typename SP::Lds) + 15) & ~(size_t)15);
    typename SP::Lds *const sw = reinterpret_cast<typename SP::Lds *>(lds_base(0u));
    __shared__ PoolIdle idle;
    const uint32_t xcc = pool_xcc_id();
    if (threadIdx.x == 0) atomicCAS(&pa->pool.ctl->t_first, 0ull, (unsigned long long)wall_clock64());
    const int wave = threadIdx.x >> 6;
    typename SP::Lds &s = sw[wave];
    if (threadIdx.x == 0) {
        idle.leave = 0u;
        idle.claims_done = 0u;
        idle.mean_calls = 0u;
    }
    SP::prepare(pa->a, s);
    if (LANE < NUM_COUNTERS) s.ctr[LANE] = 0;
    __syncthreads();
    pool_search<SP, MODE>(pa, n_calls, log_key, s, SW_BYTES + (uint32_t)wave * dyn_stride, xcc, idle, false);
}

#ifdef AZD_TU_POOL_EXT
__global__ __launch_bounds__(POOL_XCDS * 64) void k_ext_take(PoolArgs pl, uint32_t *__restrict__ out_rows, uint32_t *__restrict__ out_home,
                                                             uint32_t *__restrict__ out_n, unsigned long long *__restrict__ t0) {
    __shared__ uint32_t n_sh;
    if (threadIdx.x == 0) n_sh = 0u;
    __syncthreads();
    const uint32_t x = threadIdx.x >> 6, qmask = pl.qcap - 1u;
    PoolCtl *ctl = pl.ctl;
    uint32_t *slots = pl.eval_slots + ((size_t)POOL_XCDS + x) * pl.qcap;
    constexpr int G = 8;
    for (int tries = 0; tries < 64; ++tries) {
        const uint32_t head = ld_sc1(&ctl->evalq[1][x].head), tail = ld_sc1(&ctl->evalq[1][x].tail);
// ... 148 lines not shown
```

azdopt_amd/csrc/space_c21.inc:

```
struct WaveLds {
    uint8_t par[PARENTS_STRIDE];
    uint8_t act_parent[256];
    uint8_t act_child[256];
    unsigned long long ctr[NUM_COUNTERS];
    uint16_t seq[MAX_NODE_ACTIONS];
    uint32_t stack[PATH_STACK];
    uint64_t root_perm[4];
    uint8_t root_par[PARENTS_STRIDE];
};
__device__ __forceinline__ double *lds_pq(uint32_t dyn) { return (double *)lds_base(dyn); }
static size_t dyn_lds_bytes(int n) {
    size_t pq = (size_t)2 * (n > 2 ? n - 2 : 1) * 32 * sizeof(double);
    return CORE_DYN_BYTES > pq ? CORE_DYN_BYTES : pq;
}

__device__ __forceinline__ void build_action_table(WaveLds &s, int A) {
    for (int i = LANE; i < A; i += 64) {
        int c = 2;
        while (c * (c + 1) / 2 - 1 <= i) ++c;
        s.act_child[i] = (uint8_t)c;
        s.act_parent[i] = (uint8_t)(i - (c * (c - 1) / 2 - 1));
    }
}

// ... 149 lines not shown
    for (int guard = 0; guard < 64; ++guard) {
        uint32_t leaf = avail;
        for (int i = 1; i < n; ++i)
            if ((avail >> i) & 1u) leaf &= ~(1u << s.par[i]);
        for (int i = 1; i < n; ++i) {
            if ((leaf >> i) & 1u) {
                avail &= ~(1u << i);
                int p = s.par[i];
                if ((avail >> p) & 1u) {
                    avail &= ~(1u << p);
                    if (pairs_out && LANE == 0) {
                        pairs_out[2 * m] = p;
                        pairs_out[2 * m + 1] = i;
                    }
                    ++m;
                }
            }
        }
        if (__popc(avail) < 2) break;
    }
    return m;
}

__device__ __forceinline__ float c21_eval(float slope, double lambda1, int mu) {
    float c = (float)mu + (float)lambda1;
    float x = c - 2.0f;
    return slope * x;
}

template <int KW>
__device__ __forceinline__ void write_state_vec(const WaveLds &s, const uint64_t (&perm)[KW], int A, float *row) {
    uint64_t cur[KW];
    current_edges<KW>(s, A, cur);
#pragma unroll
    for (int w = 0; w < KW; ++w) {
        int i = w * 64 + LANE;
        if (i < A) {
            row[i] = (float)((cur[w] >> LANE) & 1ull);
            row[A + i] = (float)((perm[w] >> LANE) & 1ull);
        }
    }
}

template <int KW_>
struct C21Space {
    static constexpr int KW = KW_;
    using Lds = WaveLds;
    struct St {
        uint64_t perm[KW_];
        double lambda;
        int mu;
    };
    static size_t dyn_bytes(const Arenas &a) { return dyn_lds_bytes(a.n); }
    static size_t pool_dyn_bytes(const Arenas &a) { return dyn_lds_bytes(a.n) > (size_t)a.S * 4 ? dyn_lds_bytes(a.n) : (size_t)a.S * 4; }
    static constexpr bool POOL_EVAL_GROUPS = true;
    __device__ static __forceinline__ float *row_stage(const Arenas &, const uint32_t dyn) { return reinterpret_cast<float *>(lds_base(dyn)); }

    __device__ static __forceinline__ uint32_t key_bit(const Lds &, const uint32_t aid) { return aid; }
    __device__ static __forceinline__ uint32_t bit_action(const Lds &, const uint32_t bit) { return bit; }
    __device__ static __forceinline__ void prepare(const Arenas &a, Lds &s) { build_action_table(s, a.A); }
    __device__ static __forceinline__ void load_cur(const Arenas &a, const int t, Lds &s, const uint32_t, St &st) {
        if (LANE < PARENTS_STRIDE) s.par[LANE] = a.cur_parents[(size_t)t * PARENTS_STRIDE + LANE];
#pragma unroll
        for (int w = 0; w < KW; ++w) st.perm[w] = a.cur_perm[(size_t)t * KW + w];
        st.lambda = a.cur_lambda[t];
        st.mu = a.cur_mu[t];
    }
    static constexpr bool TWO_PHASE_LOAD = true;
    struct Raw {
        uint64_t perm[KW], root_perm;
        double lambda;
        int32_t mu;
        uint8_t par, root_par;
    };
    __device__ static __forceinline__ void load_issue(const Arenas &a, const int t, Raw &r) {
        r.par = a.cur_parents[(size_t)t * PARENTS_STRIDE + (LANE & (PARENTS_STRIDE - 1))];
        r.root_par = a.root_parents[(size_t)t * PARENTS_STRIDE + (LANE & (PARENTS_STRIDE - 1))];
#pragma unroll
        for (int w = 0; w < KW; ++w) r.perm[w] = a.cur_perm[(size_t)t * KW + w];
        r.root_perm = a.root_perm[(size_t)t * KW + (LANE < KW ? LANE : 0)];
        r.lambda = a.cur_lambda[t];
        r.mu = a.cur_mu[t];
    }
    __device__ static __forceinline__ void load_finish(Lds &s, St &st, const Raw &r) {
        if (LANE < PARENTS_STRIDE) {
            s.par[LANE] = r.par;
            s.root_par[LANE] = r.root_par;
        }
        if (LANE < KW) s.root_perm[LANE] = r.root_perm;
#pragma unroll
        for (int w = 0; w < KW; ++w) st.perm[w] = r.perm[w];
        st.lambda = r.lambda;
        st.mu = r.mu;
    }
    __device__ static __forceinline__ void load_root(const Arenas &a, const int t, Lds &s, const uint32_t, St &st) {
        if (LANE < PARENTS_STRIDE) s.par[LANE] = a.root_parents[(size_t)t * PARENTS_STRIDE + LANE];
#pragma unroll
        for (int w = 0; w < KW; ++w) st.perm[w] = a.root_perm[(size_t)t * KW + w];
    }
    __device__ static __forceinline__ void cache_root(const Arenas &a, const int t, Lds &s) {
        if (LANE < PARENTS_STRIDE) s.root_par[LANE] = a.root_parents[(size_t)t * PARENTS_STRIDE + LANE];
        if (LANE < KW) s.root_perm[LANE] = a.root_perm[(size_t)t * KW + LANE];
    }
    __device__ static __forceinline__ void load_root_cached(const Arenas &, const int, Lds &s, const uint32_t, St &st) {
        if (LANE < PARENTS_STRIDE) s.par[LANE] = s.root_par[LANE];
#pragma unroll
        for (int w = 0; w < KW; ++w) st.perm[w] = s.root_perm[w];
    }
    __device__ static __forceinline__ void store_cur(const Arenas &a, const int t, Lds &s, const uint32_t, const St &st) {
// ... 181 lines not shown
```

azdopt_amd/csrc/space_ops.h:

```cpp
#pragma once
#include "engine_types.h"

namespace azd {

struct PhaseOps {
    void (*init_roots)(const Arenas &a, const uint8_t *d_roots, const uint64_t *d_permitted, void *stream);
    void (*add_actions)(const Arenas &a, int root_mode, void *stream);
    void (*rollout)(const Arenas &a, const TolTable &tol, void *stream);
    void (*argmin)(const Arenas &a, int init_mode, void *stream);
    void (*argmin_log)(const Arenas &a, int n_calls, unsigned long long *log_key, void *stream);
    void (*observe)(const Arenas &a, uint32_t n_obs_tol, void *stream);
    void (*modify_roots)(const Arenas &a, uint64_t seed, uint64_t epoch, uint64_t first_agent, int kmin, int kmax, uint8_t *d_roots,
                         uint64_t *d_perm, uint64_t *d_slots, void *stream);
    void (*argmin_one)(const Arenas &a, int agent, uint32_t node, void *stream);
    bool (*persist_plan)(const Arenas &a, const FusedEval &ev, uint32_t *dyn_stride, size_t *dyn_bytes, const char **why);
    void (*launch_persist)(const Arenas &a, const PersistArgs *d_args, const StepLaunch &sl, uint32_t *log_node, uint32_t dyn_stride,
                           size_t dyn_bytes, void *stream);
};
struct AsyncOps {
    bool (*async_plan)(const Arenas &a, const FusedEval &ev, uint32_t *dyn_stride, size_t *dyn_bytes, const char **why);
    void (*launch_async)(const Arenas &a, const PersistArgs *d_args, const StepLaunch &sl, const float *params, const void *wpk,
                         uint32_t dyn_stride, size_t dyn_bytes, void *stream);
};
struct PoolOps {
    bool (*pool_plan)(const Arenas &a, const FusedEval &ev, PoolArgs *pool, uint32_t *dyn_stride, size_t *dyn_bytes, const char **why);
    void (*launch_pool)(const Arenas &a, const PersistArgs *d_args, const StepLaunch &sl, const float *params, const void *wpk,
                        int n_blocks, uint32_t dyn_stride, size_t dyn_bytes, void *stream);
    int (*pool_max_resident)(const Arenas &a, size_t dyn_bytes, int n_cus);
};
struct SpaceOps : PhaseOps, AsyncOps, PoolOps {};

const PhaseOps &c21_phase_ops(), &ramsey_phase_ops();
const AsyncOps &c21_async_ops(), &ramsey_async_ops();
const PoolOps &c21_pool_ops(), &ramsey_pool_ops();
const SpaceOps &ramsey64_ops(), &dense_ops();

void launch_log_candidates(const Arenas &a, unsigned long long *log_key, uint32_t *call_ctr, void *stream);
void launch_pool_resume_scan(const Arenas &a, const PoolArgs &pool, int n_calls, uint32_t *resume, void *stream);
hipError_t launch_tile_forward(const FusedEval &ev, const PoolArgs &pool, int n_rows, const float *states, float *out, void *stream);
void launch_probe_xcc(uint32_t *d_out, int n_blocks, void *stream);
void launch_hash_predictions(float *d_out, int batch, int action_dim, uint64_t seed, uint64_t first_agent,
                             uint64_t call, void *stream);
void launch_probe_cost(const uint8_t *d_parents, int n, int count, int reps, int full, double *d_lam, int *d_mu,
                       void *stream);
void launch_probe_math(const float *d_in, float *d_out, int n, void *stream);

bool dense_pool_plan(const Arenas &a, int waves, uint32_t *dyn_stride, size_t *dyn_bytes, const char **why);
void dense_launch_pool_search(const Arenas &a, const PersistArgs *d_args, const StepLaunch &sl, int n_blocks, int waves, uint32_t dyn_stride,
                              size_t dyn_bytes, void *stream);
int dense_pool_search_resident(const Arenas &a, int waves, size_t dyn_bytes);
void launch_ext_take(const PoolArgs &pool, uint32_t *rows, uint32_t *home, uint32_t *n, unsigned long long *t0, void *stream);
void launch_park(const Arenas &a, const uint32_t *resume, int n_calls, int round, int park, void *stream);
void launch_log_candidates_resume(const Arenas &a, unsigned long long *log_key, const uint32_t *resume, int n_calls, int round, void *stream);
void launch_ext_hash_rows(const PersistArgs *d_args, const uint32_t *rows, const uint32_t *n, uint32_t cap, float *h_theta, void *stream);
void launch_ext_deliver(const PoolArgs &pool, const Arenas &a, const uint32_t *rows, const uint32_t *home, const uint32_t *n, uint32_t cap,
                        const unsigned long long *t0, void *stream);

}
```

azdopt_amd/csrc/tree_core.inc:

```

#define LANE ((int)(threadIdx.x & 63))
#define WAVE_SYNC()                                              \
    do {                                                         \
        __builtin_amdgcn_fence(__ATOMIC_RELEASE, "workgroup");   \
        __builtin_amdgcn_wave_barrier();                         \
        __builtin_amdgcn_fence(__ATOMIC_ACQUIRE, "workgroup");   \
    } while (0)

#if defined(AZD_PHASE_PROFILE) || defined(AZD_WAVE_PHASES)
#define PH_NOW() ((unsigned long long)wall_clock64())
#else
#define PH_NOW() (0ull)
#endif

#define CTR_ADD(K, V)                                            \
    do {                                                         \
        if (LANE == 0) s.ctr[K] += (unsigned long long)(V);      \
    } while (0)
#define CTR_MAX(K, V)                                                                        \
    do {                                                                                     \
        if (LANE == 0 && (unsigned long long)(V) > s.ctr[K]) s.ctr[K] = (unsigned long long)(V); \
    } while (0)

#define LDS_SYNC()                                                        \
// ... 95 lines not shown
__device__ __forceinline__ int mask_count(const uint64_t (&m)[KW]) {
    int c = 0;
#pragma unroll
    for (int w = 0; w < KW; ++w) c += __popcll(m[w]);
    return c;
}
template <int KW>
__device__ __forceinline__ uint32_t key_hash(const uint64_t (&k)[KW]) {
    uint64_t h = 0x9E3779B97F4A7C15ull;
#pragma unroll
    for (int w = 0; w < KW; ++w) {
        h = (h ^ k[w]) * 0xFF51AFD7ED558CCDull;
        h ^= h >> 32;
    }
    return (uint32_t)h;
}

extern __shared__ __align__(16) double azd_dyn_lds[];
__device__ __forceinline__ char *lds_base(uint32_t dyn) { return (char *)azd_dyn_lds + dyn; }
__device__ __forceinline__ float *lds_kids(uint32_t dyn) { return (float *)lds_base(dyn); }
__device__ __forceinline__ uint32_t *lds_tmp_arc(uint32_t dyn) { return (uint32_t *)lds_base(dyn) + MAX_NODE_ACTIONS; }
__device__ __forceinline__ uint32_t *lds_fr_id(uint32_t dyn) { return (uint32_t *)lds_base(dyn); }
__device__ __forceinline__ uint32_t *lds_fr_x(uint32_t dyn) { return (uint32_t *)lds_base(dyn) + 2 * FRONTIER_CAP; }
__device__ __forceinline__ NodeRec *lds_path_recs(uint32_t dyn) { return (NodeRec *)(lds_base(dyn) + (size_t)4 * FRONTIER_CAP * sizeof(uint32_t)); }
constexpr size_t CORE_DYN_BYTES = (size_t)4 * FRONTIER_CAP * sizeof(uint32_t) + (size_t)PATH_STACK * sizeof(NodeRec);
static_assert(CORE_DYN_BYTES >= (size_t)2 * MAX_NODE_ACTIONS * sizeof(uint32_t), "selection scratch must fit the frontier region");

__device__ __forceinline__ uint64_t wave_or_u64(uint64_t v) {
    return ((uint64_t)wave_or_u32((uint32_t)(v >> 32)) << 32) | wave_or_u32((uint32_t)v);
}
__device__ __forceinline__ uint64_t splitmix(uint64_t x) {
    x += 0x9E3779B97F4A7C15ull;
    x = (x ^ (x >> 30)) * 0xBF58476D1CE4E5B9ull;
    x = (x ^ (x >> 27)) * 0x94D049BB133111EBull;
    return x ^ (x >> 31);
}
constexpr uint64_t DOMAIN_RESET_DEV = 0x72657365ull;
__device__ __forceinline__ uint64_t stream_key_dev(uint64_t seed, uint64_t domain, uint64_t agent, uint64_t draw) {
    return splitmix(splitmix(splitmix(splitmix(seed) ^ domain) ^ agent) ^ draw);
}
__device__ __forceinline__ uint32_t below_dev(uint64_t r, uint32_t n) { return (uint32_t)(((r >> 32) * (uint64_t)n) >> 32); }

typedef float azd_f32x4 __attribute__((ext_vector_type(4)));
__device__ __forceinline__ uint32_t ld_sc1(const uint32_t *p) { return __hip_atomic_load(p, __ATOMIC_RELAXED, __HIP_MEMORY_SCOPE_AGENT); }
__device__ __forceinline__ void st_sc1(uint32_t *p, uint32_t v) { __hip_atomic_store(p, v, __ATOMIC_RELAXED, __HIP_MEMORY_SCOPE_AGENT); }
__device__ __forceinline__ float ld_sc1_f32(const float *p) { return __hip_atomic_load(p, __ATOMIC_RELAXED, __HIP_MEMORY_SCOPE_AGENT); }
__device__ __forceinline__ void st_sc1_f32(float *p, float v) { __hip_atomic_store(p, v, __ATOMIC_RELAXED, __HIP_MEMORY_SCOPE_AGENT); }
__device__ __forceinline__ void st_sc1_x4(float *p, azd_f32x4 v) { asm volatile("global_store_dwordx4 %0, %1, off sc1" ::"v"(p), "v"(v) : "memory"); }
__device__ __forceinline__ azd_f32x4 ld_sc1_x4(const float *p) {
    azd_f32x4 v;
    asm volatile("global_load_dwordx4 %0, %1, off sc1\n\ts_waitcnt vmcnt(0)" : "=v"(v) : "v"(p) : "memory");
    return v;
}
#define VM_DRAIN() asm volatile("s_waitcnt vmcnt(0)" ::: "memory")

template <int KW>
__device__ __forceinline__ uint32_t ht_tag(const uint64_t (&k)[KW]) {
    const uint32_t f = key_hash<KW>(k) >> 16;
    return f == 0xFFFFu ? 0xFFFEu : f;
}
template <int KW>
__device__ __forceinline__ uint32_t ht_entry(const uint64_t (&k)[KW], const uint32_t node) { return (ht_tag<KW>(k) << 16) | (node & 0xFFFFu); }
template <int KW>
__device__ __forceinline__ uint32_t ht_lookup(const uint32_t *ht, uint32_t mask, const uint64_t *keys, const uint64_t (&k)[KW],
                              uint32_t *ins_slot) {
    const uint32_t h = key_hash<KW>(k) & mask, tag = ht_tag<KW>(k);
    for (uint32_t probe = 0; probe <= mask; probe += 64) {
        uint32_t slot = (h + probe + (uint32_t)LANE) & mask;
        const uint32_t ent = ht[slot];
        const uint32_t nd = ent & 0xFFFFu;
        bool empty = ent == NONE;
        bool match = !empty && (ent >> 16) == tag;
        if (match) {
#pragma unroll
            for (int w = 0; w < KW; ++w) match = match && (keys[(size_t)nd * KW + w] == k[w]);
        }
        uint64_t mm = __ballot(match), me = __ballot(empty);
        int fm = mm ? first_lane(mm) : 64, fe = me ? first_lane(me) : 64;
        if (fm < fe) return rdlane(nd, fm);
        if (fe < 64) {
            *ins_slot = (h + probe + (uint32_t)fe) & mask;
            return NONE;
        }
    }
    *ins_slot = NONE;
    return NONE;
}

template <int KW>
struct Agent {
    NodeRec *nodes;
    uint64_t *keys;
    ArcRec *arcs;
    PredRec *preds;
    float *pred_g;
    uint32_t *ht;
    uint32_t *fr_spill;
    uint32_t n_nodes, n_arcs, n_preds;
    uint32_t flags;
    float cand_c;
    uint32_t cand_node;
};

__device__ __forceinline__ bool node_active(const NodeRec &r) { return node_exhausted(r) < r.act_end - r.act_begin; }
__device__ __forceinline__ NodeRec uni_rec(const NodeRec &r) {
    NodeRec u;
// ... 239 lines not shown
                        const ArcRec ar = ag.arcs[e];
                        store_pair(&ag.preds[ar.pp], lw0, lw1);
                        pnt = ar.src;
                        e = ar.next_in;
                    } else pnt = NONE;
                }
            }
            fr_sync(n_nxt);
            cur = nxt;
            n_cur = n_nxt;
        }
        return;
    }
}

template <int KW>
__device__ __forceinline__ uint32_t add_arc(Agent<KW> &ag, uint32_t src, uint32_t dst, uint32_t pp, const uint32_t aid, const float g, bool creating,
                                            const NodeRec &child, const uint32_t child_begin) {
    uint32_t e = ag.n_arcs;
    if (LANE == 0) {
        ArcRec ar;
        ar.src = src;
        ar.dst = dst;
        ar.pp = pp;
        ar.next_in = creating ? NONE : child.first_in;
        ag.arcs[e] = ar;
        if (!creating) ag.nodes[dst].first_in = e;
        PredRec p;
        p.w0 = __float_as_uint(child.c_star);
        p.w1 = summary_w1(child);
        p.w2 = dst | (e << 16);
        p.w3 = aid | (child_begin << 12);
        ag.preds[pp] = p;
        ag.pred_g[pp] = g;
    }
    ag.n_arcs = e + 1;
    return e;
}

template <class SP, class = void>
struct SpaceVec16 {
    template <class... A> __device__ static __forceinline__ void write(A &&...) {}
};
template <class SP>
struct SpaceVec16<SP, decltype((void)&SP::write_vec16)> {
    template <class... A> __device__ static __forceinline__ void write(A &&...x) { SP::write_vec16(x...); }
};

template <class SP, class = void>
struct SpaceRowsDirect { static constexpr bool value = false; };
template <class SP>
struct SpaceRowsDirect<SP, decltype((void)SP::ROWS_DIRECT)> { static constexpr bool value = SP::ROWS_DIRECT; };
template <class SP, class = void>
struct SpaceDeferAct { static constexpr bool value = false; };
template <class SP>
struct SpaceDeferAct<SP, decltype((void)SP::DEFER_ACT)> { static constexpr bool value = SP::DEFER_ACT; };
template <class SP, class = void>
struct SpaceTwoPhaseLoad { static constexpr bool value = false; };
template <class SP>
struct SpaceTwoPhaseLoad<SP, decltype((void)SP::TWO_PHASE_LOAD)> { static constexpr bool value = SP::TWO_PHASE_LOAD; };
template <class SP, class = void>
struct SpaceReplayByWord { static constexpr bool value = false; };
template <class SP>
struct SpaceReplayByWord<SP, decltype((void)SP::REPLAY_BY_WORD)> { static constexpr bool value = SP::REPLAY_BY_WORD; };
template <class SP, class = void>
struct SpaceFrontierSpill { static constexpr bool value = false; };
template <class SP>
struct SpaceFrontierSpill<SP, decltype((void)SP::FRONTIER_SPILL)> { static constexpr bool value = SP::FRONTIER_SPILL; };

#ifndef AZD_TU_ASYNC
template <class SP>
__global__ __launch_bounds__(64) void k_init_roots(Arenas a, const uint8_t *__restrict__ root_bytes,
                                                   const uint64_t *__restrict__ permitted) {
    constexpr int KW = SP::KW;
    __shared__ typename SP::Lds s;
    const uint32_t dyn = 0;
    const int t = blockIdx.x;
    SP::prepare(a, s);
    WAVE_SYNC();
    typename SP::St st;
    const float c = SP::init_root(a, t, s, dyn, root_bytes, permitted, st);
    uint32_t *ht = a.ht + (size_t)t * a.ht_cap;
    for (uint32_t i = LANE; i < a.ht_cap; i += 64) ht[i] = NONE;
    WAVE_SYNC();
    uint64_t zero[KW];
#pragma unroll
    for (int w = 0; w < KW; ++w) zero[w] = 0;
    if (LANE == 0) {
        NodeRec r;
        r.c = c; r.c_star = c; r.nt_ex = 0; r.act_begin = 0; r.act_end = 0; r.first_in = NONE; r.in_src = NONE; r.in_pp = 0;
        a.nodes[(size_t)t * a.node_cap] = r;
#pragma unroll
        for (int w = 0; w < KW; ++w) {
            a.keys[((size_t)t * a.node_cap) * KW + w] = 0;
            a.cur_path[(size_t)t * KW + w] = 0;
        }
        ht[key_hash<KW>(zero) & (a.ht_cap - 1)] = ht_entry<KW>(zero, 0u);
        a.state_pos[t] = 0;
        a.n_nodes[t] = 1;
        a.n_arcs[t] = 0;
        a.n_preds[t] = 0;
        a.flags[t] = 0;
        a.cand_c[t] = c;
        a.cand_node[t] = 0;
    }
    SP::write_vec(a, s, dyn, st, a.state_vecs + (size_t)t * a.S);
    if (a.state_vecs16) SpaceVec16<SP>::write(a, s, dyn, st, a.state_vecs16 + (size_t)t * a.S16);
}

#endif
struct RolloutOut {
    uint32_t flags;
    float cand_c;
    uint32_t cand_node;
    uint32_t pos;
    float c;
    uint32_t n_preds;
    uint32_t *post_tail, *post_slots;
    uint32_t post_mask, post_word;
    unsigned long long *post_stamp;
    uint32_t posted;
    uint32_t known_live;
    uint32_t first_nact, first_pp, first_aid;
    float first_g;
};
struct FirstPick {
    uint64_t key;
    uint32_t aid;
    float g;
};
__device__ __forceinline__ void pick_note(FirstPick &f, const float v, const float g, const uint32_t idx, const uint32_t aid) {
    const uint64_t key = ((uint64_t)(~ordf(v)) << 32) | (uint64_t)(0xFFFFFFFFu - idx);
    if (key > f.key) {
        f.key = key;
        f.aid = aid;
        f.g = g;
    }
}
__device__ __forceinline__ PredRec pred_new(const uint32_t aid, const float c, const float g) {
    PredRec p;
    p.w0 = __float_as_uint(c - g);
    p.w1 = __float_as_uint(g);
    p.w2 = NONE;
    p.w3 = aid;
    return p;
}
__device__ __forceinline__ void pick_finish(const FirstPick &f, const uint32_t begin, const uint32_t cnt, RolloutOut *out) {
    const uint64_t best = wave_max_u64(f.key);
    out->first_nact = 0;
    if (best == 0ull || cnt == 0u) return;
    const uint64_t who = __ballot(f.key == best);
    out->first_aid = rdlane(f.aid, first_lane(who));
    out->first_g = rdlane_f32(f.g, first_lane(who));
    out->first_pp = begin + (0xFFFFFFFFu - (uint32_t)(best & 0xFFFFFFFFull));
    out->first_nact = cnt;
}
template <class SP, bool SC1 = false>
__device__ __forceinline__ void add_actions_agent(const Arenas &a, typename SP::Lds &s, const int t, const int root_mode, const RolloutOut *hint = nullptr,
                                  RolloutOut *pick = nullptr) {
    constexpr int KW = SP::KW;
    if (hint) {
        if (pick) pick->first_nact = 0;
        SP::template add_actions<SC1>(a, s, t, hint, pick);
        return;
    }
    if (a.flags[t] != 0) return;
    if (!root_mode) {
        uint64_t path[KW];
#pragma unroll
        for (int w = 0; w < KW; ++w) path[w] = a.cur_path[(size_t)t * KW + w];
        if (mask_empty<KW>(path)) return;
    }
    SP::template add_actions<SC1>(a, s, t, nullptr, nullptr);
}
__device__ __forceinline__ bool add_actions_fits(const Arenas &a, const int t, const uint32_t begin, const uint32_t cnt,
                                                 const uint32_t max_actions = MAX_NODE_ACTIONS) {
    uint32_t fl = 0;
    if (cnt > max_actions) fl |= FLAG_NODE_ACTIONS;
// ... 336 lines not shown
        if (out) out->flags = 1u;
        return false;
    }
    Agent<KW> ag;
    ag.nodes = a.nodes + (size_t)t * a.node_cap;
    ag.keys = a.keys + (size_t)t * a.node_cap * KW;
    ag.arcs = a.arcs + (size_t)t * a.arc_cap;
    ag.preds = a.preds + (size_t)t * a.pred_cap;
    ag.pred_g = a.pred_g + (size_t)t * a.pred_cap;
    ag.ht = a.ht + (size_t)t * a.ht_cap;
    ag.fr_spill = a.fr_spill + (size_t)t * 4u * a.node_cap;
    const uint32_t nn_v = a.n_nodes[t], na_v = a.n_arcs[t], np_v = a.n_preds[t], cn_v = a.cand_node[t];
    const float cc_v = a.cand_c[t];
    uint64_t path_v[KW];
#pragma unroll
    for (int w = 0; w < KW; ++w) path_v[w] = a.cur_path[(size_t)t * KW + w];
    const uint32_t pos_v = a.state_pos[t];
    const uint32_t stack_v = a.cur_stack[(size_t)t * PATH_STACK + (LANE & (PATH_STACK - 1))];
    typename SP::St st;
    if constexpr (SpaceTwoPhaseLoad<SP>::value) {
        typename SP::Raw raw;
        SP::load_issue(a, t, raw);
        __builtin_amdgcn_sched_barrier(0);
        SP::load_finish(s, st, raw);
    } else {
        SP::load_cur(a, t, s, dyn, st);
        SP::cache_root(a, t, s);
    }
    ag.n_nodes = uni(nn_v);
    ag.n_arcs = uni(na_v);
    ag.n_preds = uni(np_v);
    ag.flags = 0;
    ag.cand_c = __uint_as_float(uni(__float_as_uint(cc_v)));
    ag.cand_node = uni(cn_v);
    if (!DEFER && LANE < 24) s.ctr[LANE] = 0;
    uint64_t path[KW];
#pragma unroll
    for (int w = 0; w < KW; ++w) path[w] = uni64(path_v[w]);
    uint32_t pos = uni(pos_v);
    const bool layered = a.layers > 1;
    if (layered) {
        const int d0 = mask_count<KW>(path);
        for (int i = LANE; i < d0; i += 64) s.seq[i] = a.cur_seq[(size_t)t * MAX_NODE_ACTIONS + i];
    }
    {
        const int d0 = mask_count<KW>(path);
        if (LANE < PATH_STACK) s.stack[LANE] = (LANE >= 1 && LANE <= d0) ? stack_v : 0u;
    }
    WAVE_SYNC();

    bool expanded_new = false;
    float new_c = 0.f;
    bool row_out = false;
    auto emit_row = [&]() __attribute__((always_inline)) {
        if constexpr (POOL && SpaceRowsDirect<SP>::value) {
            SP::write_rows_direct(a, s, dyn, st, a.state_vecs + (size_t)t * a.S, a.state_vecs16 ? a.state_vecs16 + (size_t)t * a.S16 : nullptr);
            return;
        }
        float *row = POOL ? SP::row_stage(a, dyn) : a.state_vecs + (size_t)t * a.S;
        if (!layered) {
            SP::write_vec(a, s, dyn, st, row);
            if (!POOL && a.state_vecs16) SpaceVec16<SP>::write(a, s, dyn, st, a.state_vecs16 + (size_t)t * a.S16);
        } else {
            const int d = mask_count<KW>(path);
            const int len = d + 1 < a.layers ? d + 1 : a.layers;
            const int first = d - len + 1;
            SP::load_root(a, t, s, dyn, st);
            WAVE_SYNC();
            for (int j = 0; j <= d; ++j) {
                if (j >= first) SP::write_vec(a, s, dyn, st, row + (size_t)(j - first) * a.S_inner);
                if (j < d) SP::act(a, s, dyn, st, (uint32_t)s.seq[j]);
            }
        }
        if (POOL) {
            WAVE_SYNC();
            float *dst = a.state_vecs + (size_t)t * a.S;
            if (layered) {
                const int d = mask_count<KW>(path);
                const int len = d + 1 < a.layers ? d + 1 : a.layers;
                for (int q = LANE; q < (len * a.S_inner) >> 2; q += 64) st_sc1_x4(dst + 4 * q, *reinterpret_cast<const azd_f32x4 *>(row + 4 * q));
            } else
                for (int q = LANE; q < a.S >> 2; q += 64) st_sc1_x4(dst + 4 * q, *reinterpret_cast<const azd_f32x4 *>(row + 4 * q));
            WAVE_SYNC();
        }
    };
    uint32_t next_begin = 0, next_cnt = 0;
    bool have_next = false;
    constexpr bool DEFER_ACT = SpaceDeferAct<SP>::value;
    const bool defer_act = DEFER_ACT && !layered;
    bool stale = false;
    auto state_now = [&]() __attribute__((always_inline)) {
        if constexpr (DEFER_ACT) {
            if (stale) {
                SP::load_root_cached(a, t, s, dyn, st);
                LDS_SYNC();
                SP::act_set(a, s, dyn, st, path);
                stale = false;
            }
        }
    };
    SelCtr sc;
    sc.visited = 0; sc.selects = 0; sc.deg = 0; sc.actions = 0; sc.pairs = 0;
    const unsigned long long ph_begin = PH_NOW();
    for (uint32_t guard = 0;; ++guard) {
        if (guard > (1u << 22)) {
            ag.flags |= FLAG_LOOP_GUARD;
            break;
        }
        const unsigned long long ph_sel0 = PH_NOW();
        const bool preselected = POOL && guard == 0 && out && out->first_nact != 0;
        uint32_t r_begin = 0, nact = 0;
        bool r_active = false;
        if (preselected) {
        } else if (have_next) {
            r_begin = next_begin;
            nact = next_cnt;
            r_active = true;
        } else {
            const NodeRec rec = uni_rec(ag.nodes[pos]);
            r_begin = rec.act_begin;
            nact = rec.act_end - rec.act_begin;
            r_active = node_active(rec);
        }
        have_next = false;
        const int depth = mask_count<KW>(path);
        const uint32_t tl = depth < tol.n_tol ? tol.tol[depth] : tol.tol_default;
        int kind = 0;
        uint32_t sel_pp = 0, sel_child = 0, sel_aid = 0;
// ... 39 lines not shown
            break;
        }
        sel_pp = uni(sel_pp);
        if (layered && LANE == 0) s.seq[depth] = (uint16_t)sel_aid;
        {
            const uint32_t kb = SP::key_bit(s, sel_aid);
            path[kb >> 6] |= 1ull << (kb & 63u);
        }
        {
            uint64_t d = (uint64_t)mask_count<KW>(path);
            CTR_MAX(11, d);
        }
        if (ag.n_arcs >= a.arc_cap) {
            ag.flags |= FLAG_ARC_CAP;
            break;
        }
        uint32_t ins_slot = NONE;
        const unsigned long long ph_lk0 = PH_NOW();
        const bool set_keys = a.path_kind == PATH_SET;
        uint32_t hit = NONE;
        if (set_keys) hit = uni(ht_lookup<KW>(ag.ht, a.ht_cap - 1, ag.keys, path, &ins_slot));
        CTR_ADD(18, PH_NOW() - ph_lk0);
        bool reset_to_root = false;
        if (hit != NONE) {
            const unsigned long long ph_c0 = PH_NOW();
            const NodeRec mine = cascade_fetch<KW>(ag, s, depth);
            const NodeRec met = uni_rec(ag.nodes[hit]);
            add_arc<KW>(ag, pos, hit, sel_pp, sel_aid, sel_g, false, met, met.act_begin);
            LDS_SYNC();
            cascade<KW, SpaceFrontierSpill<SP>::value>(a, ag, s, dyn, pos, met, true, depth, mine);
            CTR_ADD(20, PH_NOW() - ph_c0);
            CTR_ADD(2, 1);
            reset_to_root = true;
        } else {
            ins_slot = uni(ins_slot);
            if (ag.n_nodes >= a.node_cap) {
                ag.flags |= FLAG_NODE_CAP;
                break;
            }
            if (set_keys && ins_slot == NONE) {
                ag.flags |= FLAG_HT_FULL;
                break;
            }

            const unsigned long long ph_n0 = PH_NOW();
            SpaceNewNode<SP>::begin(a, t, s, st, pos, sel_aid);
            if (defer_act && stale) state_now();
            else SP::act(a, s, dyn, st, sel_aid);
            bool term = false, term_known = false, post_pending = false;
            if (POOL && out && out->post_tail) {
                term = SP::terminal(a, s, dyn, st);
                term_known = true;
                if (!term) {
                    emit_row();
                    post_pending = true;
                }
            }
            auto post = [&]() __attribute__((always_inline)) {
                if (POOL && post_pending) {
                    VM_DRAIN();
                    if (LANE == 0) {
#ifdef AZD_PHASE_PROFILE
                        __hip_atomic_store(out->post_stamp, (unsigned long long)wall_clock64(), __ATOMIC_RELAXED, __HIP_MEMORY_SCOPE_AGENT);
#endif
                        const uint32_t i = atomicAdd(out->post_tail, 1u);
                        st_sc1(out->post_slots + (i & out->post_mask), out->post_word);
                    }
                    row_out = true;
                    post_pending = false;
                }
            };
            if constexpr (!SpaceRowsDirect<SP>::value) post();
            const float c_as = SpaceEvaluate<SP>::run(a, s, dyn, st, t, post);
            post();
            CTR_ADD(19, PH_NOW() - ph_n0);
            const uint32_t v = ag.n_nodes;
            NodeRec fresh;
            fresh.c = c_as; fresh.c_star = c_as; fresh.nt_ex = 0; fresh.act_begin = 0; fresh.act_end = 0; fresh.first_in = NONE; fresh.in_src = pos; fresh.in_pp = sel_pp;
            if (LANE == 0) {
                ag.nodes[v] = fresh;
#pragma unroll
                for (int w = 0; w < KW; ++w) ag.keys[(size_t)v * KW + w] = path[w];
                if (set_keys) ag.ht[ins_slot] = ht_entry<KW>(path, v);
            }
            ag.n_nodes = v + 1;
            SpaceNewNode<SP>::end(a, t, s, st, v);
            if (c_as < ag.cand_c || ag.cand_node == NONE) {
                ag.cand_c = c_as;
                ag.cand_node = v;
            }
            LDS_SYNC();
            add_arc<KW>(ag, pos, v, sel_pp, sel_aid, sel_g, true, fresh, ag.n_preds);
            LDS_SYNC();
            if (term_known ? term : SP::terminal(a, s, dyn, st)) {
                const unsigned long long ph_c0 = PH_NOW();
                cascade<KW, SpaceFrontierSpill<SP>::value>(a, ag, s, dyn, pos, fresh, false, depth, cascade_fetch<KW>(ag, s, depth));
                CTR_ADD(20, PH_NOW() - ph_c0);
                CTR_ADD(1, 1);
                reset_to_root = true;
            } else {
                pos = v;
                if (LANE == 0 && depth + 1 < PATH_STACK) s.stack[depth + 1] = v;
                new_c = c_as;
                CTR_ADD(0, 1);
                expanded_new = true;
                break;
            }
        }
        if (ag.flags) break;
        if (reset_to_root) {
            LDS_SYNC();
            if (defer_act) stale = true;
            else SP::load_root_cached(a, t, s, dyn, st);
#pragma unroll
            for (int w = 0; w < KW; ++w) path[w] = 0;
            pos = 0;
            LDS_SYNC();
        }
    }

    CTR_ADD(3, sc.visited);
    CTR_ADD(4, sc.selects);
    CTR_ADD(5, sc.deg);
    CTR_ADD(6, sc.actions);
    CTR_ADD(12, sc.pairs);
    CTR_ADD(16, PH_NOW() - ph_begin);
    CTR_MAX(21, PH_NOW() - ph_begin);
    WAVE_SYNC();
    state_now();
    if (expanded_new && !row_out) emit_row();
    if (layered) {
        const int d1 = mask_count<KW>(path);
        for (int i = LANE; i < d1; i += 64) a.cur_seq[(size_t)t * MAX_NODE_ACTIONS + i] = s.seq[i];
    }
    {
        const int d1 = mask_count<KW>(path);
        if (LANE >= 1 && LANE <= d1 && LANE < PATH_STACK) a.cur_stack[(size_t)t * PATH_STACK + LANE] = s.stack[LANE];
    }
    SP::store_cur(a, t, s, dyn, st);
    if (LANE == 0) {
#pragma unroll
        for (int w = 0; w < KW; ++w) a.cur_path[(size_t)t * KW + w] = path[w];
        a.state_pos[t] = pos;
        a.n_nodes[t] = ag.n_nodes;
        a.n_arcs[t] = ag.n_arcs;
        a.cand_c[t] = ag.cand_c;
        a.cand_node[t] = ag.cand_node;
        if (ag.flags) {
            a.flags[t] = ag.flags;
            atomicAdd(&a.status->failed, 1ull);
        }
    }
    if (out) {
        out->flags = ag.flags;
        out->cand_c = ag.cand_c;
        out->cand_node = ag.cand_node;
        out->pos = pos;
        out->c = new_c;
        out->n_preds = ag.n_preds;
        if (POOL) out->posted = row_out ? 1u : 0u;
    }
    if (!DEFER) flush_counters(a, s, t);
    return expanded_new;
}

#ifndef AZD_TU_ASYNC
template <class SP>
__global__ __launch_bounds__(64) void k_rollout(Arenas a, TolTable tol) {
    __shared__ typename SP::Lds s;
    SP::prepare(a, s);
    WAVE_SYNC();
    rollout_agent<SP>(a, tol, s, 0u, (int)blockIdx.x + a.t0);
}

#endif
static_assert(PRED_CHUNKS == 2, "selection code addresses prediction chunks 0 and 1 explicitly");

template <class SP>
__device__ void argmin_replay(const Arenas &a, typename SP::Lds &s, const uint32_t dyn, const int wt, const uint32_t win_node,
                              const int init_mode) {
    constexpr int KW = SP::KW;
    SP::prepare(a, s);
    WAVE_SYNC();
// ... 68 lines not shown
    argmin_replay<SP>(a, s, dyn, wt, win_node, init_mode);
}

template <class SP>
__global__ __launch_bounds__(64) void k_observe(Arenas a, uint32_t n_obs_tol) {
    __shared__ typename SP::Lds s;
    const uint32_t dyn = 0;
    const int t = blockIdx.x;
    const int A = a.A;
    SP::prepare(a, s);
    WAVE_SYNC();
    typename SP::St st;
    SP::load_root(a, t, s, dyn, st);
    WAVE_SYNC();
    SP::write_vec(a, s, dyn, st, a.state_vecs + (size_t)t * a.S);
    float *obs = a.obs + (size_t)t * A, *wts = a.weights + (size_t)t * A;
    for (int i = LANE; i < A; i += 64) {
        obs[i] = 0.f;
        wts[i] = 0.f;
    }
    WAVE_SYNC();
    const NodeRec *nodes = a.nodes + (size_t)t * a.node_cap;
    const PredRec *preds = a.preds + (size_t)t * a.pred_cap;
    const NodeRec root = nodes[0];
    const uint32_t nact = root.act_end - root.act_begin;
    for (uint32_t idx = LANE; idx < nact; idx += 64) {
        PredRec p = preds[root.act_begin + idx];
        if (pred_expanded(p)) {
            NodeRec cr = nodes[pred_child(p)];
            if (!node_active(cr) || node_nt(cr) >= n_obs_tol) {
                obs[pred_aid(p)] = SP::h_sa(root.c, cr.c, cr.c_star);
                wts[pred_aid(p)] = 1.0f;
            }
        }
    }
}

#endif

template <class SP>
__global__ __launch_bounds__(64) void k_argmin_log1(Arenas a, int n_calls, unsigned long long *__restrict__ log_key, PoolCtl *ctl) {
    __shared__ typename SP::Lds s;
    const uint32_t dyn = 0;
    if (ctl) {
        const uint32_t ab = ctl->abort;
        if (LANE == 0) {
            a.status->pool_abort = ab;
            a.status->pool_eval_busy = ctl->eval_busy;
            a.status->pool_search_busy = ctl->search_busy;
            a.status->pool_ticks = ctl->t_last > ctl->t_first ? ctl->t_last - ctl->t_first : 0ull;
        }
        if (ab) return;
        WAVE_SYNC();
        for (uint32_t i = LANE; i < sizeof(PoolCtl) / 4; i += 64) reinterpret_cast<uint32_t *>(ctl)[i] = 0u;
    } else if (LANE == 0) a.status->pool_abort = 0ull;
    uint32_t best = ordf(a.argmin->eval);
    int wt = -1;
    uint32_t win_node = NONE;
    unsigned long long improved = 0;
    for (int base = 0; base < n_calls; base += 64) {
        const int i = base + LANE;
        const unsigned long long k = i < n_calls ? log_key[i] : ~0ull;
        if (i < n_calls) log_key[i] = ~0ull;
        for (int j = 0; j < 64 && base + j < n_calls; ++j) {
            const unsigned long long kj = (unsigned long long)uni64(__shfl(k, j, 64));
            if (kj != ~0ull && (uint32_t)(kj >> 32) < best) {
                best = (uint32_t)(kj >> 32);
                wt = (int)((kj >> 16) & 0xFFFFull);
                win_node = (uint32_t)(kj & 0xFFFFull);
                improved += 1;
            }
        }
    }
    if (wt < 0) return;
    if (LANE == 0) atomicAdd(&a.status->improved, improved - 1);
    argmin_replay<SP>(a, s, dyn, wt, win_node, 0);
}

template <class SP>
__global__ __launch_bounds__(64) void k_argmin_one(Arenas a, int wt, uint32_t win_node) {
    __shared__ typename SP::Lds s;
    argmin_replay<SP>(a, s, 0u, wt, win_node, 1);
}

#ifndef AZD_TU_ASYNC
static __global__ __launch_bounds__(1024) void k_log_candidates(Arenas a, unsigned long long *__restrict__ log_key, uint32_t *__restrict__ call_ctr) {
    __shared__ unsigned long long s_best[16];
    const int tid = threadIdx.x;
    const int lo = a.t0, hi = a.t0 + (a.tn ? a.tn : a.B);
    unsigned long long mine = ~0ull;
    for (int t = lo + tid; t < hi; t += (int)blockDim.x) {
        const uint32_t node = a.cand_node[t];
        if (node != NONE && a.flags[t] == 0) {
            const unsigned long long key = ((unsigned long long)ordf(a.cand_c[t]) << 32) | ((unsigned long long)((uint32_t)t & 0xFFFFu) << 16) |
                                           (unsigned long long)(node & 0xFFFFu);
            mine = key < mine ? key : mine;
        }
        a.cand_node[t] = NONE;
    }
    mine = wave_min_u64(mine);
    if ((tid & 63) == 0) s_best[tid >> 6] = mine;
    __syncthreads();
    if (tid < 64) {
        unsigned long long v = tid < (int)(blockDim.x >> 6) ? s_best[tid] : ~0ull;
        v = wave_min_u64(v);
        if (tid == 0) {
            const uint32_t c = *call_ctr;
// ... 7 lines not shown
```

azdopt_amd/optimizer.py:

```python
import ctypes as C

import numpy as np

from . import _lib
from .space import ActionSet


class ArgminData:

    def __init__(self, rec, n, kw):
        self.state = dict(parents=np.array(rec.parents[:n], np.uint8), permitted=np.array(rec.permitted[:kw], np.uint64))
        m = rec.matching_size
        self.cost = dict(lambda_1=rec.lambda_1, matching=[(rec.matching[2 * i], rec.matching[2 * i + 1]) for i in range(m)])
        self.eval = np.float32(rec.eval)
        self.agent, self.node = rec.agent, rec.node


class RamseyArgminData:

    def __init__(self, rec, space):
        self.state = dict(colors=np.array(rec.colors[:space.E], np.uint8), permitted=np.array(rec.permitted[:], np.uint64))
        self.cost = dict(clique_counts=[int(x) for x in rec.totals[:space.C]])
        self.eval = np.float32(rec.eval)
        self.agent, self.node = rec.agent, rec.node
# ... 222 lines not shown
                     exhausted=np.zeros(nn, np.uint32), act_begin=np.zeros(nn, np.uint32),
                     act_end=np.zeros(nn, np.uint32), keys=np.zeros((nn, kw), np.uint64),
                     e_src=np.zeros(ne, np.uint32), e_dst=np.zeros(ne, np.uint32), e_pp=np.zeros(ne, np.uint32),
                     p_aid=np.zeros(npred, np.uint32), p_g=np.zeros(npred, np.float32), p_edge=np.zeros(npred, np.int32))
        _lib.check(self._L.azd_engine_export_tree(self._h, agent, *[_lib.ptr(getattr(t, f)) for f in TreeView.FIELDS]),
                   "export_tree")
        return t

    def get_trees(self):
        return [self.get_tree(i) for i in range(self.batch)]

    def agent_state(self, agent):
        parents = np.zeros(self.space.ROOT_BYTES, np.uint8)
        permitted = np.zeros(self.space.KEY_WORDS, np.uint64)
        path = np.zeros(self.space.KEY_WORDS, np.uint64)
        pos, lam, mu = C.c_uint32(), C.c_double(), C.c_int32()
        _lib.check(self._L.azd_engine_agent_state(self._h, agent, _lib.ptr(parents), _lib.ptr(permitted), _lib.ptr(path),
                                                  C.byref(pos), C.byref(lam), C.byref(mu)), "agent_state")
        return dict(parents=parents, permitted=permitted, path=path, state_pos=pos.value, lambda1=lam.value, matching=mu.value)

    def ramsey_argmin_any(self):
        import types
        E = self.space.E
        colors, permitted, totals = np.zeros(E, np.uint8), np.zeros((E + 63) // 64, np.uint64), np.zeros(4, np.int32)
        ev, agent, node = C.c_float(), C.c_int32(), C.c_uint32()
        _lib.check(self._L.azd_engine_ramsey_argmin_any(self._h, _lib.ptr(colors), E, _lib.ptr(permitted), len(permitted), _lib.ptr(totals),
                                                         C.byref(ev), C.byref(agent), C.byref(node)), "ramsey_argmin_any")
        return types.SimpleNamespace(colors=colors, permitted=permitted, totals=totals, eval=ev.value, agent=agent.value, node=node.value)

    def ramsey_agent_counts(self, agent):
        counts = np.zeros((self.space.C, self.space.E), np.int32)
        totals = np.zeros(4, np.int32)
        _lib.check(self._L.azd_engine_ramsey_agent_counts(self._h, agent, _lib.ptr(counts), _lib.ptr(totals)), "ramsey_agent_counts")
        return counts, totals[:self.space.C]

    def counters(self):
        out = np.zeros(_lib.CTR_COUNT, np.uint64)
        _lib.check(self._L.azd_engine_counters(self._h, _lib.ptr(out)), "counters")
        return {k: int(out[v]) for k, v in _lib.CTR.items()}

    def agent_counters(self, allow_wave_blocks=False):
        if not allow_wave_blocks and self._L.azd_engine_agent_counters_per_agent(self._h) == 0:
            raise RuntimeError("agent_counters: the pool step of the product build attributes counters to searcher waves, not agents "
                               "(use counters() for the sums, the PROFILE build or pool_step=False for per-agent values)")
        out = np.zeros((self.batch, _lib.CTR_COUNT), np.uint64)
        _lib.check(self._L.azd_engine_agent_counters(self._h, _lib.ptr(out)), "agent_counters")
        return {k: out[:, v].copy() for k, v in _lib.CTR.items()}

    def pool_groups(self):
        g, n, w = C.c_int(), C.c_int(), C.c_int()
        _lib.check(self._L.azd_engine_pool_groups(self._h, C.byref(g), C.byref(n), C.byref(w)), "pool_groups")
        return g.value, n.value, w.value

    def pool_agent_finish_ms(self):
        out = np.zeros(self.batch, np.uint64)
        _lib.check(self._L.azd_engine_pool_agent_finish(self._h, _lib.ptr(out)), "pool_agent_finish")
        return out.astype(np.float64) * 1e-5

    def set_timing(self, enabled=True):
        _lib.check(self._L.azd_engine_set_timing(self._h, int(enabled)), "set_timing")

    def timing(self):
        a, b, n = C.c_double(), C.c_double(), C.c_uint64()
        _lib.check(self._L.azd_engine_timing(self._h, C.byref(a), C.byref(b), C.byref(n)), "timing")
        return dict(rollout_ms=a.value, evaluator_ms=b.value, rollout_launches=n.value)

    def stream(self):
        return self._L.azd_engine_stream(self._h)

    STEP_FORMS = {0: "none", 1: "async", 2: "barrier", 3: "per_call", 4: "pool", 5: "per_call_graph"}

    def pool_split(self):
        a, b = C.c_int32(), C.c_int32()
        _lib.check(self._L.azd_engine_pool_split(self._h, C.byref(a), C.byref(b)), "pool_split")
        return a.value, b.value

    def pool_utilisation(self):
        a, b = C.c_double(), C.c_double()
        _lib.check(self._L.azd_engine_pool_utilisation(self._h, C.byref(a), C.byref(b)), "pool_utilisation")
        return a.value, b.value

    def step_form(self):
        form, why = C.c_int32(), C.c_char_p()
        _lib.check(self._L.azd_engine_step_form(self._h, C.byref(form), C.byref(why)), "step_form")
        return self.STEP_FORMS.get(form.value, "?"), (why.value or b"").decode()
```

include/azdopt_amd.h:

```cpp
#ifndef AZDOPT_AMD_H
#define AZDOPT_AMD_H
#include <stdint.h>
#ifdef __cplusplus
extern "C" {
#endif

typedef enum azd_status {
    AZD_OK = 0,
    AZD_ERR_INVALID_ARGUMENT = 1,
    AZD_ERR_NO_DEVICE = 2,
    AZD_ERR_HIP = 3,
    AZD_ERR_CAPACITY = 4,
    AZD_ERR_UNREACHABLE = 5,
    AZD_ERR_NO_EVALUATOR = 6,
    AZD_ERR_OUT_OF_MEMORY = 7,
    AZD_ERR_UNSUPPORTED = 8
} azd_status;

const char *azd_status_string(int status);
const char *azd_last_error(void);
int azd_version(void);
int azd_device_count(void);

#define AZD_SPACE_C21 1
// ... 186 lines not shown
int azd_engine_ramsey_wide_argmin_data(azd_engine *e, azd_ramsey_wide_argmin *out);
int azd_engine_ramsey_argmin_any(azd_engine *e, uint8_t *colors, int colors_cap, uint64_t *permitted, int permitted_words_cap,
                                 int32_t *totals, float *eval, int32_t *agent, uint32_t *node);
int azd_engine_dense_argmin_data(azd_engine *e, azd_dense_argmin *out);
int azd_engine_ramsey_agent_counts(azd_engine *e, int agent, int32_t *counts, int32_t *totals);

int azd_c21_modify_roots(azd_engine *e, uint64_t seed, uint64_t epoch, int kmin, int kmax,
                         uint8_t *parents_out, uint64_t *permitted_out);

int azd_c21_modify_roots_dev(azd_engine *e, uint64_t seed, uint64_t epoch, int kmin, int kmax,
                             uint8_t *parents_out, uint64_t *permitted_out);
int azd_engine_par_reset_trees_c21(azd_engine *e, uint64_t seed, uint64_t epoch, int kmin, int kmax);
int azd_engine_modify_roots_dev(azd_engine *e, uint64_t seed, uint64_t epoch, int kmin, int kmax,
                                uint8_t *roots_out, uint64_t *permitted_out);
int azd_engine_par_reset_trees_policy(azd_engine *e, uint64_t seed, uint64_t epoch, int kmin, int kmax);

int azd_engine_par_new_begin(azd_engine *e, const uint8_t *parents, const uint64_t *permitted);
int azd_engine_par_new_end(azd_engine *e, const float *h_theta);
int azd_engine_roll_out_begin(azd_engine *e, const uint32_t *n_as_tol, int n_tol,
                              uint32_t n_as_tol_default);
int azd_engine_roll_out_end(azd_engine *e, const float *h_theta, int *improved);
int azd_engine_reset_begin(azd_engine *e, const uint8_t *parents, const uint64_t *permitted);
int azd_engine_reset_end(azd_engine *e, const float *h_theta);
int azd_engine_observe(azd_engine *e, uint32_t n_obs_tol, float *state_vecs, float *observations,
                       float *action_weights);
int azd_engine_observe_dev(azd_engine *e, uint32_t n_obs_tol, const float **d_state_vecs,
                           const float **d_observations, const float **d_action_weights);
int azd_engine_read_state_vecs(azd_engine *e, float *state_vecs);
int azd_engine_read_predictions(azd_engine *e, float *h_theta);
int azd_engine_debug_tile_forward(azd_engine *e, const float *states, float *predictions, int rows);

int azd_engine_tree_sizes(azd_engine *e, int agent, int *n_nodes, int *n_arcs, int *n_predictions);
int azd_engine_export_tree(azd_engine *e, int agent, float *c, float *c_star, uint32_t *n_t,
                           uint32_t *exhausted, uint32_t *act_begin, uint32_t *act_end,
                           uint64_t *keys, uint32_t *arc_src, uint32_t *arc_dst, uint32_t *arc_pp,
                           uint32_t *pred_a_id, float *pred_g, int32_t *pred_arc);
int azd_engine_agent_state(azd_engine *e, int agent, uint8_t *parents, uint64_t *permitted,
                           uint64_t *path, uint32_t *state_pos, double *lambda_1,
                           int *matching_size);
int azd_engine_counters(azd_engine *e, uint64_t *out );
int azd_engine_agent_counters(azd_engine *e, uint64_t *out);
int azd_engine_agent_counters_per_agent(azd_engine *e);
int azd_engine_set_timing(azd_engine *e, int enabled);
int azd_engine_timing(azd_engine *e, double *tree_ms, double *evaluator_ms, uint64_t *tree_launches);
void *azd_engine_stream(azd_engine *e);
#define AZD_STEP_NONE 0
#define AZD_STEP_ASYNC 1
#define AZD_STEP_BARRIER 2
#define AZD_STEP_PER_CALL 3
#define AZD_STEP_POOL 4
#define AZD_STEP_PER_CALL_GRAPH 5
int azd_engine_step_form(azd_engine *e, int *form, const char **reason);
int azd_engine_pool_groups(azd_engine *e, int *members, int *groups, int *waves_per_slot);
int azd_engine_pool_agent_finish(azd_engine *e, uint64_t *ticks_out);
int azd_engine_pool_split(azd_engine *e, int *eval_wgs, int *search_wgs);
int azd_engine_pool_utilisation(azd_engine *e, double *eval_busy, double *search_busy);
int azd_debug_probe_xcc(int device, uint32_t *out, int n_blocks);
int azd_debug_hash_stream_via_evaluators(azd_evaluator *ev, int on);
int azd_debug_mlp_gradients(azd_evaluator *ev, int batch, const float *states, const float *observations,
                            const float *action_weights, float *grads_out, float *loss);

int azd_debug_probe_math(int device, const float *in, float *out, int n);
int azd_debug_probe_cost(int device, const uint8_t *parents, int n, int count, int reps, int full,
                         double *lambda_1, int *matching_size, float *ms);

int azd_debug_gemm_bf16(int device, int M, int N, int Kp, const void *d_a, const void *d_w, const float *d_bias, void *d_y, int ldy,
                        int out_bf16, int act, int reps, float *ms);

#ifdef __cplusplus
}
#endif
#endif
```

Baseline: 38.81 million.

## Post packed bit rows with ticketed records to pool evaluators for C21 single-layer

For the C21 space with a single-layer evaluator, search waves now publish each expanded state as a packed bitmask in 64-bit ticket-stamped records instead of a float row plus a slot flag. Evaluator waves poll those records and expand the bits directly into LDS, and the eval-queue polling is rewritten as a wave-wide ballot over XCD queues that drops the priority queue. The aim is to cut global-memory traffic and handshake latency between search and evaluation. In exchange it adds a record arena, extra per-granule spinning, and a host-side scan of the states in the tile-forward path.

Measured after the change: 38.32 million. 0.987x the previous value.

```diff
diff --git a/azdopt_amd/_lib.py b/azdopt_amd/_lib.py
--- a/azdopt_amd/_lib.py
+++ b/azdopt_amd/_lib.py
@@ -133,6 +133,7 @@
     sig("azd_engine_agent_counters_per_agent", C.c_int, vp)
     sig("azd_engine_pool_agent_finish", C.c_int, vp, vp)
     sig("azd_engine_pool_groups", C.c_int, vp, vp, vp, vp)
+    sig("azd_engine_pool_packed_rows", C.c_int, vp, i32p)
     sig("azd_engine_ramsey_argmin_data", C.c_int, vp, C.POINTER(RamseyArgmin))
     sig("azd_engine_ramsey_wide_argmin_data", C.c_int, vp, C.POINTER(RamseyWideArgmin))
     sig("azd_engine_ramsey_argmin_any", C.c_int, vp, vp, C.c_int, vp, C.c_int, vp, f32p, i32p, C.POINTER(C.c_uint32))
diff --git a/azdopt_amd/csrc/engine.hip b/azdopt_amd/csrc/engine.hip
--- a/azdopt_amd/csrc/engine.hip
+++ b/azdopt_amd/csrc/engine.hip
@@ -188,6 +188,9 @@
     bool pool_step = false;
     azd::PoolArgs pool{};
     size_t pool_slot_words = 0;
+    unsigned long long *d_pool_recs = nullptr;
+    size_t pool_rec_bytes = 0;
+    uint32_t pool_packed_gran = 0;
     int n_cus = 0;
     int pool_eval_wgs = 0, pool_search_wgs = 0;
     int pool_grp_g = 0, pool_grp_groups = 0, pool_grp_w = 0;
@@ -957,7 +960,7 @@
     if (e->h_win_log) (void)hipHostFree(e->h_win_log);
     if (e->h_win_flag) (void)hipHostFree(e->h_win_flag);
     if (e->d_pool) (void)hipFree(e->d_pool);
-    for (void *p : {(void *)e->d_grp_tile, (void *)e->d_grp_lds, (void *)e->d_grp_desc, (void *)e->d_grp_cnt, (void *)e->d_grp_x, (void *)e->d_grp_flag})
+    for (void *p : {(void *)e->d_grp_tile, (void *)e->d_grp_lds, (void *)e->d_grp_desc, (void *)e->d_grp_cnt, (void *)e->d_grp_x, (void *)e->d_grp_flag, (void *)e->d_pool_recs})
         if (p) (void)hipFree(p);
     if (e->call_graph) (void)hipGraphExecDestroy(e->call_graph);
     for (int i = 0; i < azd_engine::MAX_SUBS; ++i) {
@@ -1111,10 +1114,17 @@
     return false;
 }
 
+static uint32_t pool_packed_gran(const azd_engine *e, const azd::FusedEval &fe) {
+    if (e->a.space != azd::SPACE_C21 || e->a.layers > 1 || fe.kind != 3) return 0u;
+    if (const char *env = getenv("AZD_POOL_PACKED_ROWS"))
+        if (atoi(env) == 0) return 0u;
+    return 1u + ((uint32_t)e->a.S + 31u) / 32u;
+}
 static int pool_clear(azd_engine *e, const azd::PoolArgs &pool) {
     AZD_HIP(hipMemsetAsync(pool.ctl, 0, sizeof(azd::PoolCtl), e->stream));
     AZD_HIP(hipMemsetAsync(pool.ready_slots, 0, e->pool_slot_words * sizeof(uint32_t), e->stream));
     AZD_HIP(hipMemsetAsync(pool.join, 0, (size_t)e->a.B * sizeof(uint32_t), e->stream));
+    if (e->d_pool_recs) AZD_HIP(hipMemsetAsync(e->d_pool_recs, 0, e->pool_rec_bytes, e->stream));
     e->pool_clean = true;
     return AZD_OK;
 }
@@ -1593,6 +1603,27 @@
                 if (gpl.lds_bytes > dyn_bytes) dyn_bytes = gpl.lds_bytes;
             }
         }
+        pool.rec_gran = pool.grp_g == 0 ? pool_packed_gran(e, fe) : 0u;
+        if (pool.rec_gran) {
+            const size_t bytes = (size_t)2 * azd::POOL_XCDS * pool.qcap * pool.rec_gran * sizeof(unsigned long long);
+            if (bytes > e->pool_rec_bytes) {
+                AZD_HIP(hipStreamSynchronize(e->stream));
+                if (e->d_pool_recs) (void)hipFree(e->d_pool_recs);
+                e->d_pool_recs = nullptr;
+                e->pool_rec_bytes = 0;
+                const hipError_t he = hipMalloc(&e->d_pool_recs, bytes);
+                if (he != hipSuccess) {
+                    e->d_pool_recs = nullptr;
+                    const int rc = azd::hip_fail(he, "hipMalloc");
+                    azd::g_last_error = "pool step: the packed-row record arena (" + std::to_string(bytes) + " bytes) cannot be allocated: " + azd::g_last_error;
+                    return rc;
+                }
+                e->pool_rec_bytes = bytes;
+                e->pool_clean = false;
+            }
+            pool.eval_slots = reinterpret_cast<uint32_t *>(e->d_pool_recs);
+        }
+        e->pool_packed_gran = pool.rec_gran;
         pool_blocks = n_eval + n_search;
         e->pool_grp_g = pool.grp_g;
         e->pool_grp_groups = pool.grp_groups;
@@ -2357,7 +2388,9 @@
     const char *what = "hipMalloc";
     if (he == hipSuccess) he = hipMalloc(&d_out, (size_t)rows * e->a.A * 4);
     if (he == hipSuccess) what = "hipMemcpyAsync", he = hipMemcpyAsync(d_in, states, (size_t)rows * e->a.S * 4, hipMemcpyHostToDevice, e->stream);
-    if (he == hipSuccess) what = "k_tile_forward", he = azd::launch_tile_forward(fe, pool, rows, d_in, d_out, e->stream);
+    bool packed = pool_packed_gran(e, fe) != 0u;
+    for (size_t i = 0; packed && i < (size_t)rows * e->a.S; ++i) packed = states[i] == 0.0f || states[i] == 1.0f;
+    if (he == hipSuccess) what = "k_tile_forward", he = azd::launch_tile_forward(fe, pool, rows, d_in, d_out, packed ? 1 : 0, e->stream);
     if (he == hipSuccess) what = "hipMemcpyAsync", he = hipMemcpyAsync(predictions, d_out, (size_t)rows * e->a.A * 4, hipMemcpyDeviceToHost, e->stream);
     if (he == hipSuccess) what = "hipStreamSynchronize", he = hipStreamSynchronize(e->stream);
     else (void)hipStreamSynchronize(e->stream);
@@ -2559,6 +2592,11 @@
     if (search_busy) *search_busy = e->pool_util_search;
     return AZD_OK;
 }
+int azd_engine_pool_packed_rows(azd_engine *e, int *granules) {
+    if (!e || !granules) return AZD_ERR_INVALID_ARGUMENT;
+    *granules = (int)e->pool_packed_gran;
+    return AZD_OK;
+}
 int azd_engine_pool_groups(azd_engine *e, int *members, int *groups, int *waves_per_slot) {
     if (!e) return AZD_ERR_INVALID_ARGUMENT;
     if (members) *members = e->pool_grp_g;
diff --git a/azdopt_amd/csrc/engine_types.h b/azdopt_amd/csrc/engine_types.h
--- a/azdopt_amd/csrc/engine_types.h
+++ b/azdopt_amd/csrc/engine_types.h
@@ -238,6 +238,7 @@
     PoolCtl *ctl;
     uint32_t *ready_slots;
     uint32_t *eval_slots;
+    uint32_t rec_gran;
     int ready_lanes;
     int n_express;
     uint32_t express_waves;
diff --git a/azdopt_amd/csrc/pool_kernels.hip b/azdopt_amd/csrc/pool_kernels.hip
--- a/azdopt_amd/csrc/pool_kernels.hip
+++ b/azdopt_amd/csrc/pool_kernels.hip
@@ -34,7 +34,7 @@
 
 __global__ __launch_bounds__(PERSIST_WAVES * 64) void k_tile_forward(const FusedEval ev, const float *__restrict__ params, const void *__restrict__ wpk,
                                                                      const uint32_t stride, const uint32_t out_off, const int n_rows,
-                                                                     const float *__restrict__ states, float *__restrict__ out) {
+                                                                     const float *__restrict__ states, float *__restrict__ out, const int packed) {
     __shared__ uint32_t agents[PERSIST_WAVES];
     const int tid = threadIdx.x, wave = tid >> 6, first = blockIdx.x * PERSIST_WAVES;
     const int n = n_rows - first < PERSIST_WAVES ? n_rows - first : PERSIST_WAVES;
@@ -50,6 +50,18 @@
     gp.wpk = wpk;
     gp.state_vecs = states;
     gp.h_theta = out;
+    if (packed) {
+        const int W = (S + 31) >> 5;
+        for (int idx = tid; idx < n * W; idx += PERSIST_WAVES * 64) {
+            const int r = idx / W, m = idx - r * W;
+            uint32_t w = 0u;
+            for (int b = 0; b < 32; ++b) {
+                const int c = 32 * m + b;
+                if (c < S && states[(size_t)(first + r) * S + c] != 0.f) w |= 1u << b;
+            }
+            pool_expand_bits(rows.row(r), 32 * m, S16, w, ev.bf16 != 0);
+        }
+    } else
     for (int idx = tid; idx < n * S16; idx += PERSIST_WAVES * 64) {
         const int r = idx / S16, c = idx - r * S16;
         const float v = c < S ? states[(size_t)(first + r) * S + c] : 0.f;
@@ -70,12 +82,12 @@
         out[(size_t)(first + r) * A + c] = rows.out(r)[c];
     }
 }
-hipError_t launch_tile_forward(const FusedEval &ev, const PoolArgs &pool, int n_rows, const float *states, float *out, void *stream) {
+hipError_t launch_tile_forward(const FusedEval &ev, const PoolArgs &pool, int n_rows, const float *states, float *out, int packed, void *stream) {
     const size_t dyn_bytes = (size_t)pool.eval_stride * sizeof(float) * PERSIST_WAVES;
     hipError_t he = hipFuncSetAttribute((const void *)k_tile_forward, hipFuncAttributeMaxDynamicSharedMemorySize, (int)dyn_bytes);
     if (he != hipSuccess) return he;
     k_tile_forward<<<dim3((n_rows + PERSIST_WAVES - 1) / PERSIST_WAVES), dim3(PERSIST_WAVES * 64), dyn_bytes, (hipStream_t)stream>>>(
-        ev, ev.params, ev.wpk, pool.eval_stride, pool.eval_out_off, n_rows, states, out);
+        ev, ev.params, ev.wpk, pool.eval_stride, pool.eval_out_off, n_rows, states, out, packed);
     return hipGetLastError();
 }
 __global__ void k_pool_resume_scan(Arenas a, const PendRec *__restrict__ pend, const uint32_t *__restrict__ claim_next, const int n_calls,
diff --git a/azdopt_amd/csrc/pool_step.inc b/azdopt_amd/csrc/pool_step.inc
--- a/azdopt_amd/csrc/pool_step.inc
+++ b/azdopt_amd/csrc/pool_step.inc
@@ -211,7 +211,25 @@
     }
 }
 
-template <bool HASHED>
+__device__ __forceinline__ void pool_expand_bits(float *row, const int c0, const int S16, const uint32_t w, const bool bf16) {
+#pragma unroll
+    for (int q = 0; q < 8; ++q) {
+        const int c = c0 + 4 * q;
+        if (c >= S16) break;
+        const uint32_t b = w >> (4 * q);
+        if (bf16) {
+            uint2 d;
+            d.x = ((b & 1u) ? 0x3F80u : 0u) | ((b & 2u) ? 0x3F800000u : 0u);
+            d.y = ((b & 4u) ? 0x3F80u : 0u) | ((b & 8u) ? 0x3F800000u : 0u);
+            *reinterpret_cast<uint2 *>(reinterpret_cast<uint16_t *>(row) + c) = d;
+        } else {
+            azd_f32x4 v = {(b & 1u) ? 1.f : 0.f, (b & 2u) ? 1.f : 0.f, (b & 4u) ? 1.f : 0.f, (b & 8u) ? 1.f : 0.f};
+            *reinterpret_cast<azd_f32x4 *>(row + c) = v;
+        }
+    }
+}
+
+template <bool HASHED, bool ROWBITS>
 __device__ __forceinline__ void pool_eval(const PersistArgs *pa, const EvalPtrs &gp, PoolBatch &bt, const uint32_t xcc) {
     const Arenas &a = pa->a;
     const FusedEval &ev = pa->ev;
@@ -227,111 +245,149 @@
     rows.agents = bt.agent;
     unsigned long long n_batches = 0, n_rows = 0, n_tiles = 0, busy = 0, t_stage = 0, t_layers = 0, c_layers = 0;
     for (;;) {
-        if (tid == 0) {
-            uint32_t n = 0, first0 = 0, first1 = 0, cnt0 = 0, cnt1 = 0, q = 0, leave = 0;
+        if (wave == 0) {
+            static_assert(AZD_POOL_PRIORITY == 0, "pool_eval looks at evalq[1] only");
+            uint32_t n = 0, first1 = 0, q = 0, leave = 0;
             PoolWait wt;
             int fill_waits = AZD_POOL_FILL_WAIT;
             for (;;) {
-                for (uint32_t k = 0; k < (uint32_t)POOL_XCDS && n == 0u; ++k) {
-                    const uint32_t x = (xcc + k) & (uint32_t)(POOL_XCDS - 1);
-                    const uint32_t h0 = AZD_POOL_PRIORITY ? ld_sc1(&ctl->evalq[0][x].head) : 0u, t0 = AZD_POOL_PRIORITY ? ld_sc1(&ctl->evalq[0][x].tail) : 0u;
-                    const uint32_t h1 = ld_sc1(&ctl->evalq[1][x].head), t1 = ld_sc1(&ctl->evalq[1][x].tail);
-                    const int a0 = (int)(t0 - h0) > 0 ? (int)(t0 - h0) : 0, a1 = (int)(t1 - h1) > 0 ? (int)(t1 - h1) : 0;
-                    if (a0 + a1 == 0) continue;
-                    const int cap = ((int)pl.eval_rows > PERSIST_WAVES && a0 + a1 >= (int)pl.eval_rows) ? (int)pl.eval_rows : PERSIST_WAVES;
-                    if (a0 == 0 && a1 < PERSIST_WAVES && fill_waits > 0) {
+                uint32_t h1 = 0, t1 = 0;
+                if (tid < POOL_XCDS) {
+                    const uint32_t xq = (xcc + (uint32_t)tid) & (uint32_t)(POOL_XCDS - 1);
+                    h1 = ld_sc1(&ctl->evalq[1][xq].head);
+                    t1 = ld_sc1(&ctl->evalq[1][xq].tail);
+                }
+                const int a1 = (tid < POOL_XCDS && (int)(t1 - h1) > 0) ? (int)(t1 - h1) : 0;
+                const uint64_t nonempty = __ballot(a1 > 0);
+                if (nonempty) {
+                    const int pick = first_lane(nonempty);
+                    const int ap = (int)rdlane((uint32_t)a1, pick);
+                    if (ap < PERSIST_WAVES && fill_waits > 0) {
                         --fill_waits;
                         __builtin_amdgcn_s_sleep(AZD_POOL_FILL_SLEEP);
-                        k = (uint32_t)POOL_XCDS;
                         continue;
                     }
-                    uint32_t c0 = 0, c1 = 0;
-                    if (a0 > 0) {
-                        const uint32_t take = a0 < cap ? (uint32_t)a0 : (uint32_t)cap;
-                        if (atomicCAS(&ctl->evalq[0][x].head, h0, h0 + take) == h0) c0 = take;
-                    }
-                    if (a1 > 0 && c0 < (uint32_t)cap) {
-                        const uint32_t room = (uint32_t)cap - c0;
-                        const uint32_t take = (uint32_t)a1 < room ? (uint32_t)a1 : room;
-                        if (atomicCAS(&ctl->evalq[1][x].head, h1, h1 + take) == h1) c1 = take;
-                    }
-                    if (c0 + c1) {
-                        n = c0 + c1;
-                        first0 = h0;
-                        first1 = h1;
-                        cnt0 = c0;
-                        cnt1 = c1;
-                        q = x;
-                    } else k = (uint32_t)POOL_XCDS;
-                }
-                if (n) break;
-                if (ld_sc1(&ctl->done_agents) >= B || ld_sc1(&ctl->abort) != 0u) {
+                    const int cap = ((int)pl.eval_rows > PERSIST_WAVES && ap >= (int)pl.eval_rows) ? (int)pl.eval_rows : PERSIST_WAVES;
+                    const uint32_t hp = rdlane(h1, pick), take = ap < cap ? (uint32_t)ap : (uint32_t)cap;
+                    const uint32_t xp = (xcc + (uint32_t)pick) & (uint32_t)(POOL_XCDS - 1);
+                    uint32_t won = 0;
+                    if (tid == 0) won = atomicCAS(&ctl->evalq[1][xp].head, hp, hp + take) == hp ? 1u : 0u;
+                    if (uni(won)) {
+                        n = take;
+                        first1 = hp;
+                        q = xp;
+                        break;
+                    }
+                    continue;
+                }
+                uint32_t over = 0;
+                if (tid == 0) over = (ld_sc1(&ctl->done_agents) >= B || ld_sc1(&ctl->abort) != 0u) ? 1u : 0u;
+                if (uni(over)) {
                     leave = 1;
                     break;
                 }
                 __builtin_amdgcn_s_sleep(AZD_POOL_EVAL_IDLE_SLEEP);
                 if (wt.expired()) {
-                    atomicExch(&ctl->abort, 1u);
+                    if (tid == 0) atomicExch(&ctl->abort, 1u);
                     leave = 1;
                     break;
                 }
             }
-            bt.n = n;
-            bt.first[0] = first0;
-            bt.first[1] = first1;
-            bt.cnt[0] = cnt0;
-            bt.cnt[1] = cnt1;
-            bt.q = q;
-            bt.leave = leave;
+            if (tid == 0) {
+                bt.n = n;
+                bt.first[0] = 0u;
+                bt.first[1] = first1;
+                bt.cnt[0] = 0u;
+                bt.cnt[1] = n;
+                bt.q = q;
+                bt.leave = leave;
+            }
         }
         __syncthreads();
         if (bt.leave) break;
         const int n = (int)bt.n;
         const unsigned long long tb0 = (unsigned long long)wall_clock64();
-        if (tid < n) {
-            const uint32_t lane_q = (uint32_t)tid < bt.cnt[0] ? 0u : 1u;
-            const uint32_t ticket = lane_q == 0u ? bt.first[0] + (uint32_t)tid : bt.first[1] + (uint32_t)tid - bt.cnt[0];
-            uint32_t *slot = pl.eval_slots + ((size_t)lane_q * POOL_XCDS + bt.q) * pl.qcap + (ticket & qmask);
-            uint32_t v = 0;
-            PoolWait wt;
-            while ((v = ld_sc1(slot)) == 0u) {
-                __builtin_amdgcn_s_sleep(1);
-                if (wt.expired() || ld_sc1(&ctl->abort) != 0u) {
-                    atomicExch(&ctl->abort, 1u);
-                    bt.leave = 1u;
-                    break;
-                }
-            }
-            st_sc1(slot, 0u);
-            bt.agent[tid] = v ? (v & 0xFFFFFFu) - 1u : 0u;
-            bt.home[tid] = v >> 24;
+        const uint32_t G = ROWBITS ? pl.rec_gran : 0u;
+        if (G) {
+            rows.n = n;
+            if ((uint32_t)tid < (uint32_t)n * G) {
+                const uint32_t r = (uint32_t)tid / G, k = (uint32_t)tid - r * G;
+                const uint32_t ticket = bt.first[1] + r;
+                const unsigned long long *gran =
+                    reinterpret_cast<const unsigned long long *>(pl.eval_slots) + ((((uint32_t)POOL_XCDS + bt.q) * pl.qcap + (ticket & qmask)) * G + k);
+                unsigned long long v = 0;
+                bool got = true;
+                PoolWait wt;
+                while ((uint32_t)((v = ld_sc1_u64(gran)) >> 32) != ticket + 1u) {
+                    __builtin_amdgcn_s_sleep(1);
+                    if (wt.expired() || ld_sc1(&ctl->abort) != 0u) {
+                        atomicExch(&ctl->abort, 1u);
+                        bt.leave = 1u;
+                        got = false;
+                        break;
+                    }
+                }
+                const uint32_t w = got ? (uint32_t)v : 0u;
+                if (k == 0u) {
+                    bt.agent[r] = got ? (w & 0xFFFFFFu) - 1u : 0u;
+                    bt.home[r] = w >> 24;
 #ifdef AZD_PHASE_PROFILE
-            if (v) {
-                unsigned long long *st = pl.stamp + bt.agent[tid];
-                atomicAdd(&a.counters[(size_t)bt.agent[tid] * NUM_COUNTERS + 24], (unsigned long long)wall_clock64() - __hip_atomic_load(st, __ATOMIC_RELAXED, __HIP_MEMORY_SCOPE_AGENT));
-            }
-#endif
+                    if (got) {
+                        unsigned long long *st = pl.stamp + bt.agent[r];
+                        atomicAdd(&a.counters[(size_t)bt.agent[r] * NUM_COUNTERS + 24], (unsigned long long)wall_clock64() - __hip_atomic_load(st, __ATOMIC_RELAXED, __HIP_MEMORY_SCOPE_AGENT));
+                    }
+#endif
+                } else pool_expand_bits(rows.row((int)r), (int)(32u * (k - 1u)), S16, w, ev.bf16 != 0);
+            }
+        } else {
+            if (tid < n) {
+                const uint32_t lane_q = (uint32_t)tid < bt.cnt[0] ? 0u : 1u;
+                const uint32_t ticket = lane_q == 0u ? bt.first[0] + (uint32_t)tid : bt.first[1] + (uint32_t)tid - bt.cnt[0];
+                uint32_t *slot = pl.eval_slots + ((size_t)lane_q * POOL_XCDS + bt.q) * pl.qcap + (ticket & qmask);
+                uint32_t v = 0;
+                PoolWait wt;
+                while ((v = ld_sc1(slot)) == 0u) {
+                    __builtin_amdgcn_s_sleep(1);
+                    if (wt.expired() || ld_sc1(&ctl->abort) != 0u) {
+                        atomicExch(&ctl->abort, 1u);
+                        bt.leave = 1u;
+                        break;
+                    }
+                }
+                st_sc1(slot, 0u);
+                bt.agent[tid] = v ? (v & 0xFFFFFFu) - 1u : 0u;
+                bt.home[tid] = v >> 24;
+#ifdef AZD_PHASE_PROFILE
+                if (v) {
+                    unsigned long long *st = pl.stamp + bt.agent[tid];
+                    atomicAdd(&a.counters[(size_t)bt.agent[tid] * NUM_COUNTERS + 24], (unsigned long long)wall_clock64() - __hip_atomic_load(st, __ATOMIC_RELAXED, __HIP_MEMORY_SCOPE_AGENT));
+                }
+#endif
+            }
+            __syncthreads();
+            if (bt.leave) break;
+            rows.n = n;
+            if (hashed) pool_hash_rows(ev, pl, bt, rows, n, A);
+            else {
+                const int q4 = S16 >> 2;
+                for (int idx = tid; idx < n * q4; idx += PERSIST_WAVES * 64) {
+                    const int r = idx / q4, c4 = idx - r * q4;
+                    azd_f32x4 v = {0.f, 0.f, 0.f, 0.f};
+                    if (4 * c4 < S) v = ld_sc1_x4(gp.state_vecs + (size_t)bt.agent[r] * S + 4 * c4);
+                    if (ev.bf16) {
+                        uint16_t *d = reinterpret_cast<uint16_t *>(rows.row(r)) + 4 * c4;
+                        d[0] = (uint16_t)bf16_bits(v[0]);
+                        d[1] = (uint16_t)bf16_bits(v[1]);
+                        d[2] = (uint16_t)bf16_bits(v[2]);
+                        d[3] = (uint16_t)bf16_bits(v[3]);
+                    } else *reinterpret_cast<azd_f32x4 *>(rows.row(r) + 4 * c4) = v;
+                }
+            }
         }
         __syncthreads();
-        if (bt.leave) break;
-        rows.n = n;
-        if (hashed) pool_hash_rows(ev, pl, bt, rows, n, A);
-        else {
-            const int q4 = S16 >> 2;
-            for (int idx = tid; idx < n * q4; idx += PERSIST_WAVES * 64) {
-                const int r = idx / q4, c4 = idx - r * q4;
-                azd_f32x4 v = {0.f, 0.f, 0.f, 0.f};
-                if (4 * c4 < S) v = ld_sc1_x4(gp.state_vecs + (size_t)bt.agent[r] * S + 4 * c4);
-                if (ev.bf16) {
-                    uint16_t *d = reinterpret_cast<uint16_t *>(rows.row(r)) + 4 * c4;
-                    d[0] = (uint16_t)bf16_bits(v[0]);
-                    d[1] = (uint16_t)bf16_bits(v[1]);
-                    d[2] = (uint16_t)bf16_bits(v[2]);
-                    d[3] = (uint16_t)bf16_bits(v[3]);
-                } else *reinterpret_cast<azd_f32x4 *>(rows.row(r) + 4 * c4) = v;
-            }
-        }
-        __syncthreads();
+        if constexpr (ROWBITS) {
+            if (bt.leave) break;
+        }
         const unsigned long long tb1 = (unsigned long long)wall_clock64();
         const unsigned long long cb1 = (unsigned long long)__builtin_amdgcn_s_memtime();
         for (int l = 0; l < L; ++l) {
@@ -688,8 +744,11 @@
     PoolCtl *ctl = pl.ctl;
     constexpr bool HASHED = (MODE & 1) != 0, WINDOW = (MODE & 2) != 0;
     const uint32_t B = (uint32_t)a.B, qmask = pl.qcap - 1u;
+    const uint32_t wave_u = uni(threadIdx.x >> 6);
     uint32_t *rslots[2] = {pl.ready_slots + (size_t)xcc * pl.qcap, pl.ready_slots + ((size_t)POOL_XCDS + xcc) * pl.qcap};
-    uint32_t *eslots[2] = {pl.eval_slots + (size_t)xcc * pl.qcap, pl.eval_slots + ((size_t)POOL_XCDS + xcc) * pl.qcap};
+    const uint32_t rec_gran = (SpaceRowBits<SP>::value && !HASHED) ? pl.rec_gran : 0u;
+    const size_t eslot_words = rec_gran ? 2u * (size_t)rec_gran : 1u;
+    uint32_t *eslots[2] = {pl.eval_slots + (size_t)xcc * pl.qcap * eslot_words, pl.eval_slots + ((size_t)POOL_XCDS + xcc) * pl.qcap * eslot_words};
     for (;;) {
 #ifdef AZD_WAVE_PHASES
         const unsigned long long wp_take0 = PH_NOW();
@@ -806,6 +865,7 @@
             }
             RolloutOut ro;
             ro.post_tail = nullptr;
+            if constexpr (SpaceRowBits<SP>::value) ro.post_mask = 0u;
             ro.posted = 0u;
             ro.known_live = first.first_nact != 0u ? 1u : 0u;
             ro.first_nact = first.first_nact;
@@ -838,7 +898,7 @@
                 }
                 ro.post_tail = early ? &ctl->evalq[lane_q][xcc].tail : nullptr;
                 ro.post_slots = eslots[lane_q];
-                ro.post_mask = qmask;
+                ro.post_mask = qmask | (rec_gran ? POST_PACKED : 0u);
                 ro.post_word = (t + 1u) | ((xcc | behind | 0x40u) << 24);
                 ro.post_stamp = pl.stamp + t;
                 if (HASHED && LANE == 0) st_sc1(pl.post_call + t, call);
@@ -879,13 +939,30 @@
                 WAVE_SYNC();
                 POOL_FLUSH_PER_AGENT(a, s, (int)t);
                 VM_DRAIN();
+                bool packed_late = false;
+                if constexpr (SpaceRowBits<SP>::value && !HASHED) {
+                    if (rec_gran && uni(ro.posted) == 0u) {
+                        uint32_t i = 0u;
+                        if (LANE == 0) {
+#ifdef AZD_PHASE_PROFILE
+                            __hip_atomic_store(pl.stamp + t, (unsigned long long)wall_clock64(), __ATOMIC_RELAXED, __HIP_MEMORY_SCOPE_AGENT);
+#endif
+                            i = atomicAdd(&ctl->evalq[lane_q][xcc].tail, 1u);
+                        }
+                        i = uni(i);
+                        post_packed<SP>(a, dyn, eslots[lane_q], i & qmask, (t + 1u) | ((xcc | behind) << 24), i);
+                        packed_late = true;
+                    }
+                }
                 if (LANE == 0) {
                     if (!ro.posted) {
+                      if (!packed_late) {
 #ifdef AZD_PHASE_PROFILE
                         __hip_atomic_store(pl.stamp + t, (unsigned long long)wall_clock64(), __ATOMIC_RELAXED, __HIP_MEMORY_SCOPE_AGENT);
 #endif
                         const uint32_t i = atomicAdd(&ctl->evalq[lane_q][xcc].tail, 1u);
                         st_sc1(eslots[lane_q] + (i & qmask), (t + 1u) | ((xcc | behind) << 24));
+                      }
                     }
                     else if (atomicAdd(&pl.join[t], 1u) & 1u) {
 #ifdef AZD_PHASE_PROFILE
@@ -924,17 +1001,18 @@
 #ifndef AZD_PHASE_PROFILE
     WAVE_SYNC();
 #ifdef AZD_WAVE_PHASES
-    if ((LANE == 24 || LANE == 28) && s.ctr[LANE]) atomicAdd(&a.counters[(size_t)((blockIdx.x * PERSIST_WAVES + (threadIdx.x >> 6)) % B) * NUM_COUNTERS + LANE], s.ctr[LANE]);
-#endif
-    if (LANE < 24) {
-        const unsigned long long v = s.ctr[LANE];
-        unsigned long long *ctr = a.counters + (size_t)((blockIdx.x * PERSIST_WAVES + (threadIdx.x >> 6)) % B) * NUM_COUNTERS;
-        if (LANE == 10 || LANE == 11 || LANE == 21) atomicMax(&ctr[LANE], v);
-        else if (v) atomicAdd(&ctr[LANE], v);
+    if ((LANE == 24 || LANE == 28) && s.ctr[LANE]) atomicAdd(&a.counters[(size_t)((blockIdx.x * PERSIST_WAVES + wave_u) % B) * NUM_COUNTERS + LANE], s.ctr[LANE]);
+#endif
+    const int tl = opaque_lane();
+    if (tl < 24) {
+        const unsigned long long v = s.ctr[tl];
+        unsigned long long *ctr = a.counters + (size_t)((blockIdx.x * PERSIST_WAVES + wave_u) % B) * NUM_COUNTERS;
+        if (tl == 10 || tl == 11 || tl == 21) atomicMax(&ctr[tl], v);
+        else if (v) atomicAdd(&ctr[tl], v);
     }
 #endif
 #ifdef AZD_PHASE_PROFILE
-    if (LANE == 0 && s.ctr[28]) atomicAdd(&a.counters[(size_t)((blockIdx.x * PERSIST_WAVES + (threadIdx.x >> 6)) % B) * NUM_COUNTERS + 28], s.ctr[28]);
+    if (LANE == 0 && s.ctr[28]) atomicAdd(&a.counters[(size_t)((blockIdx.x * PERSIST_WAVES + wave_u) % B) * NUM_COUNTERS + 28], s.ctr[28]);
 #endif
 }
 
@@ -961,7 +1039,7 @@
                 return;
             }
         }
-        pool_eval<(MODE & 1) != 0>(pa, gp, bt, xcc);
+        pool_eval<(MODE & 1) != 0, SpaceRowBits<SP>::value && (MODE & 1) == 0>(pa, gp, bt, xcc);
         return;
     }
     const int wave = threadIdx.x >> 6;
diff --git a/azdopt_amd/csrc/space_c21.inc b/azdopt_amd/csrc/space_c21.inc
--- a/azdopt_amd/csrc/space_c21.inc
+++ b/azdopt_amd/csrc/space_c21.inc
@@ -225,9 +225,28 @@
         int mu;
     };
     static size_t dyn_bytes(const Arenas &a) { return dyn_lds_bytes(a.n); }
-    static size_t pool_dyn_bytes(const Arenas &a) { return dyn_lds_bytes(a.n) > (size_t)a.S * 4 ? dyn_lds_bytes(a.n) : (size_t)a.S * 4; }
+    static size_t pool_dyn_bytes(const Arenas &a) {
+        const size_t row = (size_t)a.S * 4 + (size_t)((a.S + 63) / 64) * 8;
+        return dyn_lds_bytes(a.n) > row ? dyn_lds_bytes(a.n) : row;
+    }
     static constexpr bool POOL_EVAL_GROUPS = true;
     __device__ static __forceinline__ float *row_stage(const Arenas &, const uint32_t dyn) { return reinterpret_cast<float *>(lds_base(dyn)); }
+    static constexpr bool ROW_BITS = true;
+    __device__ static __forceinline__ void stage_row_bits(const Arenas &a, const uint32_t dyn) {
+        const float *row = row_stage(a, dyn);
+        unsigned long long *words = reinterpret_cast<unsigned long long *>(lds_base(dyn + (uint32_t)a.S * 4u));
+#pragma unroll 1
+        for (int j = 0; 64 * j < a.S; ++j) {
+            const int i = 64 * j + LANE;
+            const float f = i < a.S ? row[i] : 0.f;
+            const unsigned long long bits = __ballot(f != 0.f);
+            if (LANE == 0) words[j] = bits;
+        }
+    }
+    __device__ static __forceinline__ uint32_t row_bits_word(const Arenas &a, const uint32_t dyn, const int m) {
+        const uint32_t *words = reinterpret_cast<const uint32_t *>(lds_base(dyn + (uint32_t)a.S * 4u));
+        return (m >= 0 && m < ((a.S + 31) >> 5)) ? words[m] : 0u;
+    }
 
     __device__ static __forceinline__ uint32_t key_bit(const Lds &, const uint32_t aid) { return aid; }
     __device__ static __forceinline__ uint32_t bit_action(const Lds &, const uint32_t bit) { return bit; }
diff --git a/azdopt_amd/csrc/space_ops.h b/azdopt_amd/csrc/space_ops.h
--- a/azdopt_amd/csrc/space_ops.h
+++ b/azdopt_amd/csrc/space_ops.h
@@ -37,7 +37,7 @@
 
 void launch_log_candidates(const Arenas &a, unsigned long long *log_key, uint32_t *call_ctr, void *stream);
 void launch_pool_resume_scan(const Arenas &a, const PoolArgs &pool, int n_calls, uint32_t *resume, void *stream);
-hipError_t launch_tile_forward(const FusedEval &ev, const PoolArgs &pool, int n_rows, const float *states, float *out, void *stream);
+hipError_t launch_tile_forward(const FusedEval &ev, const PoolArgs &pool, int n_rows, const float *states, float *out, int packed, void *stream);
 void launch_probe_xcc(uint32_t *d_out, int n_blocks, void *stream);
 void launch_hash_predictions(float *d_out, int batch, int action_dim, uint64_t seed, uint64_t first_agent,
                              uint64_t call, void *stream);
diff --git a/azdopt_amd/csrc/tree_core.inc b/azdopt_amd/csrc/tree_core.inc
--- a/azdopt_amd/csrc/tree_core.inc
+++ b/azdopt_amd/csrc/tree_core.inc
@@ -171,6 +171,8 @@
     asm volatile("global_load_dwordx4 %0, %1, off sc1\n\ts_waitcnt vmcnt(0)" : "=v"(v) : "v"(p) : "memory");
     return v;
 }
+__device__ __forceinline__ unsigned long long ld_sc1_u64(const unsigned long long *p) { return __hip_atomic_load(p, __ATOMIC_RELAXED, __HIP_MEMORY_SCOPE_AGENT); }
+__device__ __forceinline__ void st_sc1_u64(unsigned long long *p, unsigned long long v) { __hip_atomic_store(p, v, __ATOMIC_RELAXED, __HIP_MEMORY_SCOPE_AGENT); }
 #define VM_DRAIN() asm volatile("s_waitcnt vmcnt(0)" ::: "memory")
 
 template <int KW>
@@ -516,6 +518,10 @@
 template <class SP>
 struct SpaceRowsDirect<SP, decltype((void)SP::ROWS_DIRECT)> { static constexpr bool value = SP::ROWS_DIRECT; };
 template <class SP, class = void>
+struct SpaceRowBits { static constexpr bool value = false; };
+template <class SP>
+struct SpaceRowBits<SP, decltype((void)SP::ROW_BITS)> { static constexpr bool value = SP::ROW_BITS; };
+template <class SP, class = void>
 struct SpaceDeferAct { static constexpr bool value = false; };
 template <class SP>
 struct SpaceDeferAct<SP, decltype((void)SP::DEFER_ACT)> { static constexpr bool value = SP::DEFER_ACT; };
@@ -588,6 +594,17 @@
     uint32_t first_nact, first_pp, first_aid;
     float first_g;
 };
+constexpr uint32_t POST_PACKED = 0x80000000u;
+template <class SP>
+__device__ __forceinline__ void post_packed(const Arenas &a, const uint32_t dyn, uint32_t *recs, const uint32_t slot, const uint32_t word,
+                                            const uint32_t ticket) {
+    const uint32_t G = 1u + (((uint32_t)a.S + 31u) >> 5);
+    const uint32_t bits = SP::row_bits_word(a, dyn, LANE - 1);
+    const uint32_t w = LANE == 0 ? word : bits;
+    if ((uint32_t)LANE < G)
+        st_sc1_u64(reinterpret_cast<unsigned long long *>(recs) + (slot * G + (uint32_t)LANE), (unsigned long long)w | ((unsigned long long)(ticket + 1u) << 32));
+}
+
 struct FirstPick {
     uint64_t key;
     uint32_t aid;
@@ -1030,7 +1047,16 @@
     bool expanded_new = false;
     float new_c = 0.f;
     bool row_out = false;
-    auto emit_row = [&]() __attribute__((always_inline)) {
+    auto copy_row = [&]() __attribute__((always_inline)) {
+        if constexpr (POOL && SpaceRowBits<SP>::value) {
+            const float *row = SP::row_stage(a, dyn);
+            float *dst = a.state_vecs + (size_t)t * a.S;
+            for (int q = LANE; q < a.S >> 2; q += 64) st_sc1_x4(dst + 4 * q, *reinterpret_cast<const azd_f32x4 *>(row + 4 * q));
+            WAVE_SYNC();
+        }
+    };
+    const bool row_packed = POOL && SpaceRowBits<SP>::value && out && (out->post_mask & POST_PACKED) != 0u;
+    auto emit_row = [&](const bool to_memory) __attribute__((always_inline)) {
         if constexpr (POOL && SpaceRowsDirect<SP>::value) {
             SP::write_rows_direct(a, s, dyn, st, a.state_vecs + (size_t)t * a.S, a.state_vecs16 ? a.state_vecs16 + (size_t)t * a.S16 : nullptr);
             return;
@@ -1052,6 +1078,13 @@
         }
         if (POOL) {
             WAVE_SYNC();
+            if constexpr (POOL && SpaceRowBits<SP>::value) {
+                if (row_packed) {
+                    SP::stage_row_bits(a, dyn);
+                    WAVE_SYNC();
+                }
+                if (!to_memory) return;
+            }
             float *dst = a.state_vecs + (size_t)t * a.S;
             if (layered) {
                 const int d = mask_count<KW>(path);
@@ -1197,12 +1230,29 @@
                 term = SP::terminal(a, s, dyn, st);
                 term_known = true;
                 if (!term) {
-                    emit_row();
+                    emit_row(!row_packed);
                     post_pending = true;
                 }
             }
             auto post = [&]() __attribute__((always_inline)) {
                 if (POOL && post_pending) {
+                    if constexpr (POOL && SpaceRowBits<SP>::value) {
+                        if (row_packed) {
+                            uint32_t i = 0;
+                            if (LANE == 0) {
+#ifdef AZD_PHASE_PROFILE
+                                __hip_atomic_store(out->post_stamp, (unsigned long long)wall_clock64(), __ATOMIC_RELAXED, __HIP_MEMORY_SCOPE_AGENT);
+#endif
+                                i = atomicAdd(out->post_tail, 1u);
+                            }
+                            i = uni(i);
+                            post_packed<SP>(a, dyn, out->post_slots, i & out->post_mask & ~POST_PACKED, out->post_word, i);
+                            copy_row();
+                            row_out = true;
+                            post_pending = false;
+                            return;
+                        }
+                    }
                     VM_DRAIN();
                     if (LANE == 0) {
 #ifdef AZD_PHASE_PROFILE
@@ -1273,7 +1323,7 @@
     CTR_MAX(21, PH_NOW() - ph_begin);
     WAVE_SYNC();
     state_now();
-    if (expanded_new && !row_out) emit_row();
+    if (expanded_new && !row_out) emit_row(true);
     if (layered) {
         const int d1 = mask_count<KW>(path);
         for (int i = LANE; i < d1; i += 64) a.cur_seq[(size_t)t * MAX_NODE_ACTIONS + i] = s.seq[i];
@@ -1448,7 +1498,13 @@
         }
         if (ab) return;
         WAVE_SYNC();
-        for (uint32_t i = LANE; i < sizeof(PoolCtl) / 4; i += 64) reinterpret_cast<uint32_t *>(ctl)[i] = 0u;
+        constexpr uint32_t q0 = (uint32_t)(__builtin_offsetof(PoolCtl, evalq) / 4), q1 = q0 + (uint32_t)(sizeof(PoolQ) * 2 * POOL_XCDS / 4);
+        for (uint32_t i = LANE; i < sizeof(PoolCtl) / 4; i += 64)
+            if (i < q0 || i >= q1) reinterpret_cast<uint32_t *>(ctl)[i] = 0u;
+        if (LANE < 2 * POOL_XCDS) {
+            PoolQ &q = ctl->evalq[LANE / POOL_XCDS][LANE % POOL_XCDS];
+            q.head = q.tail;
+        }
     } else if (LANE == 0) a.status->pool_abort = 0ull;
     uint32_t best = ordf(a.argmin->eval);
     int wt = -1;
diff --git a/azdopt_amd/optimizer.py b/azdopt_amd/optimizer.py
--- a/azdopt_amd/optimizer.py
+++ b/azdopt_amd/optimizer.py
@@ -298,6 +298,11 @@
         _lib.check(self._L.azd_engine_pool_groups(self._h, C.byref(g), C.byref(n), C.byref(w)), "pool_groups")
         return g.value, n.value, w.value
 
+    def pool_packed_rows(self):
+        g = C.c_int32()
+        _lib.check(self._L.azd_engine_pool_packed_rows(self._h, C.byref(g)), "pool_packed_rows")
+        return g.value
+
     def pool_agent_finish_ms(self):
         out = np.zeros(self.batch, np.uint64)
         _lib.check(self._L.azd_engine_pool_agent_finish(self._h, _lib.ptr(out)), "pool_agent_finish")
diff --git a/include/azdopt_amd.h b/include/azdopt_amd.h
--- a/include/azdopt_amd.h
+++ b/include/azdopt_amd.h
@@ -262,6 +262,7 @@
 #define AZD_STEP_PER_CALL_GRAPH 5
 int azd_engine_step_form(azd_engine *e, int *form, const char **reason);
 int azd_engine_pool_groups(azd_engine *e, int *members, int *groups, int *waves_per_slot);
+int azd_engine_pool_packed_rows(azd_engine *e, int *granules);
 int azd_engine_pool_agent_finish(azd_engine *e, uint64_t *ticks_out);
 int azd_engine_pool_split(azd_engine *e, int *eval_wgs, int *search_wgs);
 int azd_engine_pool_utilisation(azd_engine *e, double *eval_busy, double *search_busy);
```
